# swusjask/kzg-snark

Hardware: AMD Instinct MI355X
Metric: KZG G1 commits/sec (INTT 2^20 + commit 2^20, BLS12-381) (higher is better)
Workload: dtype integer: 13x30-bit limbs in u32 (381-bit Fp), 9x29-bit limbs (255-bit Fr), 64-bit multiply-add; 1 GPU; degree-2^20 INTT + KZG commit, bls12_381, 2^20-point SRS, uniform Fr scalars, batch of 4 polynomials per GPU per step; log_n=20, curve=bls12_381, batch=4, window_bits=20

## Files before the change

### kzg_snark_amd/csrc/api.hip

```cpp
#include "internal.h"
#include "g1_words.h"
#include "msm.h"
#include "../../include/kzg_mi355x.h"
#include <cstdio>
#include <cstring>
#include <new>

struct kzg_ctx {
  kzg::Ctx c;
};
struct kzg_srs {
  kzg::Srs* s;
};
struct kzg_domain_table {
  kzg::DomainTable* t;
};

namespace kzg {
int device_any_nonzero(Ctx* c, const uint32_t* d_words, size_t from, size_t to, bool* out);
}

namespace kzg {

int set_err(Ctx* c, int code, const char* what, hipError_t e) {
  if (c) {
    c->err = what ? what : "";
    if (e != hipSuccess) {
      c->err += ": ";
      c->err += hipGetErrorString(e);
    }
  }
  return code;
}

ProfScope::ProfScope(Ctx* ctx, const char* name, hipStream_t stream) : c(ctx) {
  if (!c->prof_on) return;
  st = stream ? stream : c->stream;
  for (auto& sp : c->prof)
    if (sp.name == name) { span = &sp; break; }
  if (!span) {
    c->prof.reserve(64);
    c->prof.push_back(ProfSpan{name, {}, 0, 0});
    span = &c->prof.back();
  }
  if (hipEventCreate(&e0) != hipSuccess || hipEventCreate(&e1) != hipSuccess) { span = nullptr; return; }
  hipEventRecord(e0, st);
}
ProfScope::~ProfScope() {
  if (!span) return;
  hipEventRecord(e1, st);
  span->pending.emplace_back(e0, e1);
}

int ensure_buf(Ctx* c, DevBuf& b, size_t bytes) {
  if (b.cap >= bytes) return KZG_OK;
  if (b.p) {
    KZG_HIP(c, hipStreamSynchronize(c->stream));
    KZG_HIP(c, hipFree(b.p));
    b.p = nullptr;
    b.cap = 0;
  }
  hipError_t e = hipMalloc(&b.p, bytes);
  if (e != hipSuccess) {
    b.p = nullptr;
    return set_err(c, KZG_ERR_ALLOC, "hipMalloc", e);
  }
  b.cap = bytes;
  return KZG_OK;
}

}

namespace kzg {
template <class C>
static int g1_sum_t(const uint64_t* xy, const uint8_t* inf, size_t n, uint64_t* out_xy, uint8_t* out_inf) {
  using F = typename C::Fp;
  const uint32_t* w = reinterpret_cast<const uint32_t*>(xy);
  XYZZ<C> acc = Ec<C>::infinity();
  for (size_t i = 0; i < n; ++i) {
    if (inf && inf[i]) continue;
    Fe<F> x, y;
    if (!import_affine<C>(w + i * 2 * F::NW, w + i * 2 * F::NW + F::NW, x, y)) return KZG_ERR_ARG;
    acc = Ec<C>::madd(acc, x, y);
  }
  *out_inf = affine_to_words<C>(Ec<C>::to_affine(acc), reinterpret_cast<uint32_t*>(out_xy));
  return KZG_OK;
}
}

using namespace kzg;

#define KZG_ENTER(bad)                           \
  if (!ctx || (bad)) return KZG_ERR_ARG;         \
  Ctx* c = &ctx->c;                              \
  KZG_HIP(c, hipSetDevice(c->device))

static int adopt_srs(int rc, Srs* s, kzg_srs** out) {
  if (rc == KZG_OK) *out = new kzg_srs{s};
  return rc;
}

static int stage_host(Ctx* c, const void* src, size_t bytes, void** d) {
  int rc = ensure_buf(c, c->io, bytes ? bytes : 32);
  if (rc) return rc;
  if (bytes) KZG_HIP(c, hipMemcpyAsync(c->io.p, src, bytes, hipMemcpyHostToDevice, c->stream));
  *d = c->io.p;
  return KZG_OK;
}

extern "C" {

int kzg_g1_sum(int curve_id, const uint64_t* xy, const uint8_t* inf, size_t n, uint64_t* out_xy, uint8_t* out_inf) {
  if ((n && !xy) || !out_xy || !out_inf) return KZG_ERR_ARG;
  if (curve_id == KZG_CURVE_BN254) return g1_sum_t<Bn254>(xy, inf, n, out_xy, out_inf);
  if (curve_id == KZG_CURVE_BLS12_381) return g1_sum_t<Bls12_381>(xy, inf, n, out_xy, out_inf);
  return KZG_ERR_ARG;
}

int kzg_abi_version(void) { return 1; }

int kzg_fp_limbs(int curve_id) {
  if (curve_id == KZG_CURVE_BN254) return 4;
  if (curve_id == KZG_CURVE_BLS12_381) return 6;
  return 0;
}

int kzg_ctx_create(int curve_id, int device_id, kzg_ctx** out) {
  if (!out) return KZG_ERR_ARG;
  *out = nullptr;
  if (curve_id != KZG_CURVE_BN254 && curve_id != KZG_CURVE_BLS12_381) return KZG_ERR_ARG;
  int ndev = 0;
  if (hipGetDeviceCount(&ndev) != hipSuccess || ndev <= 0 || device_id < 0 || device_id >= ndev)
    return KZG_ERR_NODEV;
  if (hipSetDevice(device_id) != hipSuccess) return KZG_ERR_NODEV;
  kzg_ctx* h = new (std::nothrow) kzg_ctx();
  if (!h) return KZG_ERR_ALLOC;
  h->c.curve = curve_id;
  h->c.device = device_id;
  if (hipStreamCreateWithFlags(&h->c.stream, hipStreamNonBlocking) != hipSuccess) {
    delete h;
    return KZG_ERR_HIP;
  }
  h->c.own_stream = true;
  *out = h;
  return KZG_OK;
}

void kzg_ctx_destroy(kzg_ctx* ctx) {
  if (!ctx) return;
  Ctx* c = &ctx->c;
  hipSetDevice(c->device);
  hipDeviceSynchronize();
  ntt_free_domains(c);
  msm_free_work(c);
  for (DevBuf* b : {&c->ntt_scratch, &c->io, &c->scan_tmp, &c->lagr_tmp, &c->dom_tmp, &c->ver_tmp, &c->rec_tmp,
                    &c->vpt_tmp, &c->pair_tmp, &c->gmul_tmp,
                    &c->poly_tmp[0], &c->poly_tmp[1], &c->poly_tmp[2], &c->poly_tmp[3]})
    hipFree(b->p);
  hipFree(c->clk_probe);
  if (c->eval_lens_pin) hipHostFree(c->eval_lens_pin);
  if (c->eval_lens_ev) hipEventDestroy(c->eval_lens_ev);
  for (auto s : c->aux_streams) hipStreamDestroy(s);
  for (auto e : c->aux_events) hipEventDestroy(e);
  if (c->own_stream && c->stream) hipStreamDestroy(c->stream);
  delete ctx;
}

const char* kzg_last_error(const kzg_ctx* ctx) { return ctx ? ctx->c.err.c_str() : "null context"; }

int kzg_ctx_set_stream(kzg_ctx* ctx, void* hip_stream) {
  KZG_ENTER(false);
  if (hip_stream) {
    const uintptr_t hv = reinterpret_cast<uintptr_t>(hip_stream);
    const bool alias = hip_stream == static_cast<void*>(hipStreamLegacy) || hip_stream == static_cast<void*>(hipStreamPerThread);
    if (!alias && (hv < 65536 || (hv & 7)))
      return set_err(c, KZG_ERR_ARG, "kzg_ctx_set_stream: not a stream handle (small integer or misaligned value)");
    if (c->own_stream && c->stream) {
      KZG_HIP(c, hipStreamSynchronize(c->stream));
      KZG_HIP(c, hipStreamDestroy(c->stream));
    }
    c->stream = hip_stream == static_cast<void*>(hipStreamLegacy) ? nullptr : static_cast<hipStream_t>(hip_stream);
    c->own_stream = false;
  } else if (!c->own_stream) {
    KZG_HIP(c, hipStreamCreateWithFlags(&c->stream, hipStreamNonBlocking));
    c->own_stream = true;
  }
  return KZG_OK;
}

int kzg_ctx_set_tuning(kzg_ctx* ctx, const char* key, int64_t value) {
  if (!ctx || !key) return KZG_ERR_ARG;
  Ctx* c = &ctx->c;
  const std::string k(key);
  if (k == "ntt_tile_log") {
    if (value != 0 && (value < 8 || value > 12)) return set_err(c, KZG_ERR_ARG, "ntt_tile_log: 0 or 8..12");
    c->tune_ntt_tile_log = (int)value;
  } else if (k == "open_tile_threads") {
    if (value != 0 && value != 128 && value != 256) return set_err(c, KZG_ERR_ARG, "open_tile_threads: 0, 128 or 256");
    c->tune_open_tb = (int)value;
  } else if (k == "open_direct_tiles") {
    if (value < 0 || value > (1 << 20)) return set_err(c, KZG_ERR_ARG, "open_direct_tiles: 0 .. 2^20");
    c->tune_open_direct_max = (int)value;
  } else if (k == "open_domain_chunk") {
    if (value < 0 || value > 1024) return set_err(c, KZG_ERR_ARG, "open_domain_chunk: 0 .. 1024");
    c->tune_open_domain_chunk = (int)value;
  } else if (k == "open_cosets_chunk") {
    if (value < 0 || value > 1024) return set_err(c, KZG_ERR_ARG, "open_cosets_chunk: 0 .. 1024");
    c->tune_open_cosets_chunk = (int)value;
  } else if (k == "open_cosets_group") {
    if (value < 0 || value > 5) return set_err(c, KZG_ERR_ARG, "open_cosets_group: 0 .. 5");
    c->tune_open_cosets_group = (int)value;
  } else if (k == "recover_chunk") {
    if (value < 0 || value > 1024) return set_err(c, KZG_ERR_ARG, "recover_chunk: 0 .. 1024");
    c->tune_recover_chunk = (int)value;
  } else if (k == "eval_batch_chunk") {
    if (value < 0 || value > 65535) return set_err(c, KZG_ERR_ARG, "eval_batch_chunk: 0 .. 65535");
    c->tune_eval_batch_chunk = (int)value;
  } else {
    return set_err(c, KZG_ERR_ARG, "kzg_ctx_set_tuning: unknown key");
  }
  return KZG_OK;
}

int kzg_ctx_synchronize(kzg_ctx* ctx) {
  if (!ctx) return KZG_ERR_ARG;
  Ctx* c = &ctx->c;
  KZG_HIP(c, hipStreamSynchronize(c->stream));
  return KZG_OK;
}

int kzg_ntt_device(kzg_ctx* ctx, void* d_data, uint32_t log_n, const uint64_t w[4], int inverse,
                   uint32_t batch) {
  KZG_ENTER(!d_data || !w);
  return ntt_run_device(c, static_cast<uint32_t*>(d_data), log_n, reinterpret_cast<const uint32_t*>(w),
                        inverse ? 1 : 0, batch);
}

int kzg_ntt_columns_device(kzg_ctx* ctx, void* d_data, uint32_t log_n, const uint64_t w[4], int inverse,
                           uint64_t n_cols, uint64_t col_base) {
  KZG_ENTER(!d_data || !w);
  return ntt_partial_device(c, static_cast<uint32_t*>(d_data), log_n, reinterpret_cast<const uint32_t*>(w),
                            inverse ? 1 : 0, 0, n_cols, col_base);
}

int kzg_ntt_rows_device(kzg_ctx* ctx, void* d_data, uint32_t log_n, const uint64_t w[4], int inverse,
                        uint64_t n_rows) {
  KZG_ENTER(!d_data || !w);
  return ntt_partial_device(c, static_cast<uint32_t*>(d_data), log_n, reinterpret_cast<const uint32_t*>(w),
                            inverse ? 1 : 0, 1, n_rows, 0);
}

int kzg_ntt_rows_twist_device(kzg_ctx* ctx, void* d_data, uint32_t log_n, const uint64_t w[4], int inverse,
                              uint64_t n_rows, uint64_t row_base) {
  KZG_ENTER(!d_data || !w);
  return ntt_partial_device(c, static_cast<uint32_t*>(d_data), log_n, reinterpret_cast<const uint32_t*>(w),
                            inverse ? 1 : 0, 2, n_rows, row_base);
}

int kzg_ntt_columns_plain_device(kzg_ctx* ctx, void* d_data, uint32_t log_n, const uint64_t w[4], int inverse,
                                 uint64_t n_cols) {
  KZG_ENTER(!d_data || !w);
  return ntt_partial_device(c, static_cast<uint32_t*>(d_data), log_n, reinterpret_cast<const uint32_t*>(w),
                            inverse ? 1 : 0, 3, n_cols, 0);
}

int kzg_ntt_rows_exchange_device(kzg_ctx* ctx, const void* d_src, void* d_dst, uint32_t log_n, const uint64_t w[4],
                                 int inverse, uint64_t n_rows, uint32_t world, int blocked_out) {
  KZG_ENTER(!d_src || !d_dst || !w);
  return ntt_rows_exchange_device(c, static_cast<const uint32_t*>(d_src), static_cast<uint32_t*>(d_dst), log_n,
                                  reinterpret_cast<const uint32_t*>(w), inverse ? 1 : 0, n_rows, world, blocked_out);
}

int kzg_ntt(kzg_ctx* ctx, uint64_t* data, uint32_t log_n, const uint64_t w[4], int inverse) {
  KZG_ENTER(!data || !w);
  if (log_n > 24) return set_err(c, KZG_ERR_ARG, "kzg_ntt: log_n > 24 not supported");
  const size_t bytes = (size_t)32 << log_n;
  void* d = nullptr;
  int rc = stage_host(c, data, bytes, &d);
  if (rc) return rc;
  rc = ntt_run_device(c, static_cast<uint32_t*>(d), log_n, reinterpret_cast<const uint32_t*>(w), inverse ? 1 : 0, 1);
  if (rc) return rc;
  KZG_HIP(c, hipMemcpyAsync(data, d, bytes, hipMemcpyDeviceToHost, c->stream));
  KZG_HIP(c, hipStreamSynchronize(c->stream));
  return KZG_OK;
}

int kzg_fft_ff_any_device(kzg_ctx* ctx, void* d_data, size_t n, const uint64_t w[4], int inverse) {
  KZG_ENTER(!d_data || !w);
  if (n && !(n & (n - 1))) {
    uint32_t log_n = 0;
    while ((1ull << log_n) < n) ++log_n;
    return ntt_run_device(c, static_cast<uint32_t*>(d_data), log_n, reinterpret_cast<const uint32_t*>(w),
                          inverse ? 1 : 0, 1);
  }
  return fft_ragged_device(c, static_cast<uint32_t*>(d_data), n, reinterpret_cast<const uint32_t*>(w), inverse ? 1 : 0);
}

int kzg_fft_ff_any(kzg_ctx* ctx, uint64_t* data, size_t n, const uint64_t w[4], int inverse) {
  KZG_ENTER(!data || !w);
  if (n == 0 || n > ((size_t)1 << 24)) return set_err(c, KZG_ERR_ARG, "kzg_fft_ff_any: length must be in [1, 2^24]");
  const size_t bytes = n * 32;
  void* d = nullptr;
  int rc = stage_host(c, data, bytes, &d);
  if (rc) return rc;
  rc = kzg_fft_ff_any_device(ctx, d, n, w, inverse);
  if (rc) return rc;
  KZG_HIP(c, hipMemcpyAsync(data, d, bytes, hipMemcpyDeviceToHost, c->stream));
  KZG_HIP(c, hipStreamSynchronize(c->stream));
  return KZG_OK;
}

int kzg_srs_load_g1(kzg_ctx* ctx, const uint64_t* xy, const uint8_t* inf, size_t n, kzg_srs** out) {
  KZG_ENTER(!xy || !out);
  *out = nullptr;
  Srs* s = nullptr;
  const int rc = srs_load(c, xy, inf, n, &s);
  return adopt_srs(rc, s, out);
}

int kzg_srs_generate_range(kzg_ctx* ctx, const uint64_t tau[4], size_t start, size_t n, kzg_srs** out) {
  KZG_ENTER(!tau || !out);
  *out = nullptr;
  Srs* s = nullptr;
  const int rc = srs_generate(c, tau, start, n, &s);
  return adopt_srs(rc, s, out);
}

int kzg_srs_generate_strided(kzg_ctx* ctx, const uint64_t tau[4], size_t start, size_t n, size_t run_len,
                             size_t inner_stride, size_t outer_stride, kzg_srs** out) {
  KZG_ENTER(!tau || !out || run_len == 0);
  *out = nullptr;
  Srs* s = nullptr;
  const int rc = srs_generate(c, tau, start, n, &s, run_len, inner_stride, outer_stride);
  return adopt_srs(rc, s, out);
}

int kzg_srs_generate(kzg_ctx* ctx, const uint64_t tau[4], size_t n, kzg_srs** out) {
  return kzg_srs_generate_range(ctx, tau, 0, n, out);
}

int kzg_srs_export(kzg_ctx* ctx, const kzg_srs* srs, size_t start, size_t count, uint64_t* xy, uint8_t* inf) {
  KZG_ENTER(!srs || !xy || !inf);
  return srs_export(c, srs->s, start, count, xy, inf);
}

int kzg_srs_load_g1_compressed(kzg_ctx* ctx, const uint8_t* bytes, size_t n, int check_subgroup, kzg_srs** out) {
  KZG_ENTER(!bytes || !out);
  *out = nullptr;
  Srs* s = nullptr;
  const int rc = srs_load_g1_compressed(c, bytes, n, check_subgroup, &s);
  return adopt_srs(rc, s, out);
}

int kzg_srs_export_compressed(kzg_ctx* ctx, const kzg_srs* srs, size_t start, size_t count, uint8_t* out_bytes) {
  KZG_ENTER(!srs || (count && !out_bytes));
  if (srs->s->curve != c->curve) return set_err(c, KZG_ERR_ARG, "SRS belongs to another curve");
  return srs_export_compressed(c, srs->s, start, count, out_bytes);
}

int kzg_g1_compress(kzg_ctx* ctx, const uint64_t* xy, const uint8_t* inf, size_t n, uint8_t* out_bytes) {
  KZG_ENTER(n && (!xy || !out_bytes));
  return g1_compress(c, xy, inf, n, out_bytes);
}

int kzg_g1_decompress(kzg_ctx* ctx, const uint8_t* bytes, size_t n, int check_subgroup, uint64_t* out_xy,
                      uint8_t* out_inf, uint8_t* out_status) {
  KZG_ENTER(n && (!bytes || !out_xy || !out_inf || !out_status));
  return g1_decompress(c, bytes, n, check_subgroup, out_xy, out_inf, out_status);
}

int kzg_g1_decompress_device(kzg_ctx* ctx, const void* d_bytes, size_t n, int check_subgroup, void* d_xy, void* d_inf,
                             void* d_status) {
  KZG_ENTER(n && (!d_bytes || !d_xy || !d_inf || !d_status));
  return g1_decompress_device(c, d_bytes, n, check_subgroup, d_xy, d_inf, d_status);
}

int kzg_g1_check_subgroup(kzg_ctx* ctx, const uint64_t* xy, const uint8_t* inf, size_t n, uint8_t* out_status) {
  KZG_ENTER(n && (!xy || !out_status));
  return g1_check_subgroup(c, xy, inf, n, out_status);
}

int kzg_g2_compress(kzg_ctx* ctx, const uint64_t* xy, const uint8_t* inf, size_t n, uint8_t* out_bytes) {
  KZG_ENTER(n && (!xy || !out_bytes));
  return g2_compress(c, xy, inf, n, out_bytes);
}

int kzg_g2_decompress(kzg_ctx* ctx, const uint8_t* bytes, size_t n, int check_subgroup, uint64_t* out_xy,
                      uint8_t* out_inf, uint8_t* out_status) {
  KZG_ENTER(n && (!bytes || !out_xy || !out_inf || !out_status));
  return g2_decompress(c, bytes, n, check_subgroup, out_xy, out_inf, out_status);
}

int kzg_g2_decompress_device(kzg_ctx* ctx, const void* d_bytes, size_t n, int check_subgroup, void* d_xy, void* d_inf,
                             void* d_status) {
  KZG_ENTER(n && (!d_bytes || !d_xy || !d_inf || !d_status));
  return g2_decompress_device(c, d_bytes, n, check_subgroup, d_xy, d_inf, d_status);
}

int kzg_g2_check_subgroup(kzg_ctx* ctx, const uint64_t* xy, const uint8_t* inf, size_t n, uint8_t* out_status) {
  KZG_ENTER(n && (!xy || !out_status));
  return g2_check_subgroup(c, xy, inf, n, out_status);
}

int kzg_g1_mul_each(kzg_ctx* ctx, const uint64_t* xy, const uint8_t* inf, size_t n, const uint64_t* scalars,
                    uint64_t* out_xy, uint8_t* out_inf) {
  KZG_ENTER(n && (!xy || !scalars || !out_xy || !out_inf));
  return g1_mul_each(c, xy, inf, n, reinterpret_cast<const uint32_t*>(scalars), nullptr, nullptr, out_xy, out_inf);
}

int kzg_g1_mul_each_device(kzg_ctx* ctx, const void* d_xy, const void* d_inf, size_t n, const void* d_scalars,
                           void* d_out_xy, void* d_out_inf) {
  KZG_ENTER(n && (!d_xy || !d_scalars || !d_out_xy || !d_out_inf));
  return g1_mul_each_device(c, d_xy, d_inf, n, d_scalars, d_out_xy, d_out_inf);
}

int kzg_g1_mul_powers(kzg_ctx* ctx, const uint64_t* xy, const uint8_t* inf, size_t n, const uint64_t s[4],
                      const uint64_t c0[4], uint64_t* out_xy, uint8_t* out_inf) {
  KZG_ENTER(!s || !c0 || (n && (!xy || !out_xy || !out_inf)));
  return g1_mul_each(c, xy, inf, n, nullptr, reinterpret_cast<const uint32_t*>(s), reinterpret_cast<const uint32_t*>(c0),
                     out_xy, out_inf);
}

int kzg_srs_mul_powers(kzg_ctx* ctx, const kzg_srs* srs, const uint64_t s[4], const uint64_t c0[4], kzg_srs** out) {
  KZG_ENTER(!srs || !s || !c0 || !out);
  *out = nullptr;
  if (srs->s->curve != c->curve) return set_err(c, KZG_ERR_ARG, "SRS belongs to another curve");
  Srs* key = nullptr;
  const int rc = srs_mul_powers(c, srs->s, reinterpret_cast<const uint32_t*>(s), reinterpret_cast<const uint32_t*>(c0), &key);
  return adopt_srs(rc, key, out);
}

int kzg_g2_mul_each(kzg_ctx* ctx, const uint64_t* xy, const uint8_t* inf, size_t n, const uint64_t* scalars,
                    uint64_t* out_xy, uint8_t* out_inf) {
  KZG_ENTER(n && (!xy || !scalars || !out_xy || !out_inf));
  return g2_mul_each(c, xy, inf, n, reinterpret_cast<const uint32_t*>(scalars), nullptr, nullptr, out_xy, out_inf);
}

int kzg_g2_mul_powers(kzg_ctx* ctx, const uint64_t* xy, const uint8_t* inf, size_t n, const uint64_t s[4],
                      const uint64_t c0[4], uint64_t* out_xy, uint8_t* out_inf) {
  KZG_ENTER(!s || !c0 || (n && (!xy || !out_xy || !out_inf)));
  return g2_mul_each(c, xy, inf, n, nullptr, reinterpret_cast<const uint32_t*>(s), reinterpret_cast<const uint32_t*>(c0),
                     out_xy, out_inf);
}

int kzg_g2_lincomb(kzg_ctx* ctx, const uint64_t* xy, const uint8_t* inf, size_t n, const uint64_t* scalars,
                   uint64_t* out_xy, uint8_t* out_inf) {
  KZG_ENTER(!out_xy || !out_inf || (n && (!xy || !scalars)));
  return g2_lincomb(c, xy, inf, n, reinterpret_cast<const uint32_t*>(scalars), nullptr, nullptr, out_xy, out_inf);
}

int kzg_g2_lincomb_powers(kzg_ctx* ctx, const uint64_t* xy, const uint8_t* inf, size_t n, const uint64_t s[4],
                          const uint64_t c0[4], uint64_t* out_xy, uint8_t* out_inf) {
  KZG_ENTER(!s || !c0 || !out_xy || !out_inf || (n && !xy));
  return g2_lincomb(c, xy, inf, n, nullptr, reinterpret_cast<const uint32_t*>(s), reinterpret_cast<const uint32_t*>(c0),
                    out_xy, out_inf);
}

int kzg_pairing_check(kzg_ctx* ctx, const uint64_t* g1_xy, const uint8_t* g1_inf, const uint64_t* g2_xy,
                      const uint8_t* g2_inf, size_t m, size_t k, uint8_t* out_status) {
  KZG_ENTER(m && (!g1_xy || !g2_xy || !out_status));
  return pairing_product(c, g1_xy, g1_inf, g2_xy, g2_inf, m, k, nullptr, out_status);
}

int kzg_pairing_product(kzg_ctx* ctx, const uint64_t* g1_xy, const uint8_t* g1_inf, const uint64_t* g2_xy,
                        const uint8_t* g2_inf, size_t m, size_t k, uint64_t* out_gt, uint8_t* out_status) {
  KZG_ENTER(m && (!g1_xy || !g2_xy || !out_gt || !out_status));
  return pairing_product(c, g1_xy, g1_inf, g2_xy, g2_inf, m, k, out_gt, out_status);
}

int kzg_pairing_gt_multiple(int curve) { return pairing_gt_multiple(curve); }

int kzg_blob_to_fr(kzg_ctx* ctx, uint32_t log_n, const uint8_t* blobs, size_t b, int bit_reversed, uint64_t* out_vals,
                   uint8_t* out_status) {
  KZG_ENTER(b && (!blobs || !out_vals || !out_status));
  return blob_to_fr(c, log_n, blobs, b, bit_reversed, out_vals, out_status);
}

int kzg_blob_to_fr_device(kzg_ctx* ctx, uint32_t log_n, const void* d_blobs, size_t b, int bit_reversed, void* d_vals,
                          void* d_status) {
  KZG_ENTER(b && (!d_blobs || !d_vals || !d_status));
  return blob_to_fr_device(c, log_n, d_blobs, b, bit_reversed, d_vals, d_status);
}

int kzg_fr_to_blob(kzg_ctx* ctx, uint32_t log_n, const uint64_t* vals, size_t b, int bit_reversed, uint8_t* out_bytes,
                   uint8_t* out_status) {
  KZG_ENTER(b && (!vals || !out_bytes || !out_status));
  return fr_to_blob(c, log_n, vals, b, bit_reversed, out_bytes, out_status);
}

int kzg_fr_to_blob_device(kzg_ctx* ctx, uint32_t log_n, const void* d_vals, size_t b, int bit_reversed, void* d_bytes,
                          void* d_status) {
  KZG_ENTER(b && (!d_vals || !d_bytes || !d_status));
  return fr_to_blob_device(c, log_n, d_vals, b, bit_reversed, d_bytes, d_status);
}

int kzg_blob_challenges(kzg_ctx* ctx, uint32_t log_n, const uint8_t* blobs, const uint8_t* commitments, size_t b,
                        uint64_t* out_z) {
  KZG_ENTER(b && (!blobs || !commitments || !out_z));
  return blob_challenges(c, log_n, blobs, commitments, b, out_z);
}

int kzg_blob_challenges_device(kzg_ctx* ctx, uint32_t log_n, const void* d_blobs, const void* d_commitments, size_t b,
                               void* d_z) {
  KZG_ENTER(b && (!d_blobs || !d_commitments || !d_z));
  return blob_challenges_device(c, log_n, d_blobs, d_commitments, b, d_z);
}

size_t kzg_srs_size(const kzg_srs* srs) { return srs ? srs->s->n : 0; }

void kzg_srs_free(kzg_srs* srs) {
  if (!srs) return;
  srs_free(srs->s);
  delete srs;
}

int kzg_commit_device(kzg_ctx* ctx, const kzg_srs* srs, const void* d_scalars, const size_t* lens, size_t n_polys,
                      size_t stride, uint64_t* out_xy, uint8_t* out_inf) {
  KZG_ENTER(!srs || !lens || !out_xy || !out_inf || (n_polys && !d_scalars));
  return commit_device(c, srs->s, static_cast<const uint32_t*>(d_scalars), lens, n_polys, stride, out_xy, out_inf);
}

int kzg_commit_device_async(kzg_ctx* ctx, const kzg_srs* srs, const void* d_scalars, const size_t* lens,
                            size_t n_polys, size_t stride, uint64_t* out_xy, uint8_t* out_inf) {
  KZG_ENTER(!srs || !lens || !out_xy || !out_inf || (n_polys && !d_scalars));
  return commit_device(c, srs->s, static_cast<const uint32_t*>(d_scalars), lens, n_polys, stride, out_xy, out_inf,
                       false);
}

int kzg_commit_flush(kzg_ctx* ctx) {
  KZG_ENTER(false);
  return commit_flush(c);
}

int kzg_commit(kzg_ctx* ctx, const kzg_srs* srs, const uint64_t* scalars, const size_t* lens, size_t n_polys,
               size_t stride, uint64_t* out_xy, uint8_t* out_inf) {
  KZG_ENTER(!srs || !lens || !out_xy || !out_inf || (n_polys && stride && !scalars));
  const size_t bytes = n_polys * stride * 32;
  int rc = ensure_buf(c, c->io, bytes ? bytes : 32);
  if (rc) return rc;
  const size_t fpw = (c->curve == 0 ? Bn254::Fp::NW : Bls12_381::Fp::NW) / 2;
  auto* io = static_cast<uint32_t*>(c->io.p);
  for (size_t p = 0; p < n_polys; ++p) {
    if (lens[p] > srs->s->n) return set_err(c, KZG_ERR_DEGREE, "polynomial longer than the commitment key");
    if (lens[p] > stride) return set_err(c, KZG_ERR_ARG, "kzg_commit: lens[p] > stride");
  }
  for (size_t p = 0; p < n_polys && rc == KZG_OK; ++p) {
    if (lens[p])
      rc = KZG_HIP_RC(c, hipMemcpyAsync(io + p * stride * 8, scalars + p * stride * 4, lens[p] * 32,
                                        hipMemcpyHostToDevice, c->stream));
    if (rc == KZG_OK)
      rc = commit_device(c, srs->s, io + p * stride * 8, lens + p, 1, stride, out_xy + p * 2 * fpw, out_inf + p, false);
  }
  const int rc2 = commit_flush(c);
  return rc ? rc : rc2;
}

int kzg_open_device(kzg_ctx* ctx, const kzg_srs* srs, const void* d_polys, const size_t* lens, size_t k,
                    size_t stride, const uint64_t z[4], const uint64_t xi[4], uint64_t* out_xy, uint8_t* out_inf,
                    uint64_t* eval_out) {
  KZG_ENTER(!srs || !z || !xi || !out_xy || !out_inf || (k && (!lens || !d_polys)));
  uint32_t* d_quot = nullptr;
  size_t qlen = 0;
  uint64_t ev[4];
  int rc = open_quotient_device(c, static_cast<const uint32_t*>(d_polys), lens, k, stride,
                                reinterpret_cast<const uint32_t*>(z), reinterpret_cast<const uint32_t*>(xi), &d_quot,
                                &qlen, ev);
  if (rc) return rc;
  if (eval_out) memcpy(eval_out, ev, 32);
  const size_t srs_n = srs->s->n;
  if (qlen > srs_n) {
    bool nz = false;
    rc = device_any_nonzero(c, d_quot, srs_n, qlen, &nz);
    if (rc) return rc;
    if (nz) return set_err(c, KZG_ERR_DEGREE, "witness polynomial longer than the commitment key");
    qlen = srs_n;
  }
  return commit_device(c, srs->s, d_quot, &qlen, 1, qlen ? qlen : 1, out_xy, out_inf);
}

int kzg_open_device_async(kzg_ctx* ctx, const kzg_srs* srs, const void* d_polys, const size_t* lens, size_t k,
                          size_t stride, const uint64_t z[4], const uint64_t xi[4], uint64_t* out_xy, uint8_t* out_inf,
                          uint64_t* eval_out) {
  KZG_ENTER(!srs || !z || !xi || !out_xy || !out_inf || !eval_out || (k && (!lens || !d_polys)));
  uint32_t* d_quot = nullptr;
  size_t qlen = 0;
  int rc = open_quotient_device(c, static_cast<const uint32_t*>(d_polys), lens, k, stride,
                                reinterpret_cast<const uint32_t*>(z), reinterpret_cast<const uint32_t*>(xi), &d_quot,
                                &qlen, eval_out, false);
  if (rc) return rc;
  if (!d_quot) {
    memset(out_xy, 0, (size_t)kzg_fp_limbs(c->curve) * 16);
    *out_inf = 1;
    memset(eval_out, 0, 32);
    return KZG_OK;
  }
  const size_t srs_n = srs->s->n;
  if (qlen > srs_n) {
    bool nz = false;
    rc = device_any_nonzero(c, d_quot, srs_n, qlen, &nz);
    if (rc) return rc;
    if (nz) return set_err(c, KZG_ERR_DEGREE, "witness polynomial longer than the commitment key");
    qlen = srs_n;
  }
  return commit_device(c, srs->s, d_quot, &qlen, 1, qlen ? qlen : 1, out_xy, out_inf, false, d_quot - 8,
                       eval_out);
}

int kzg_open(kzg_ctx* ctx, const kzg_srs* srs, const uint64_t* polys, const size_t* lens, size_t k, size_t stride,
             const uint64_t z[4], const uint64_t xi[4], uint64_t* out_xy, uint8_t* out_inf, uint64_t* eval_out) {
  KZG_ENTER(!srs || !z || !xi || !out_xy || !out_inf || (k && (!lens || !polys)));
  void* d = nullptr;
  if (int rc = stage_host(c, polys, k * stride * 32, &d)) return rc;
  return kzg_open_device(ctx, srs, d, lens, k, stride, z, xi, out_xy, out_inf, eval_out);
}

int kzg_open_points_device(kzg_ctx* ctx, const kzg_srs* srs, const void* d_polys, const size_t* lens, size_t k,
                           size_t stride, const uint64_t* points, size_t t, const uint64_t* weights, void* d_quot,
                           uint64_t* out_xy, uint8_t* out_inf) {
  KZG_ENTER(!srs || !out_xy || !out_inf || (k && (!lens || !d_polys)) || (t && !points) || (k && t && !weights));
  uint32_t* d_q = nullptr;
  size_t qlen = 0;
  int rc = open_points_quotient_device(c, static_cast<const uint32_t*>(d_polys), lens, k, stride,
                                       reinterpret_cast<const uint32_t*>(points), t,
                                       reinterpret_cast<const uint32_t*>(weights), &d_q, &qlen);
  if (rc) return rc;
  if (!d_q) {
    memset(out_xy, 0, (size_t)kzg_fp_limbs(c->curve) * 16);
    *out_inf = 1;
    return KZG_OK;
  }
  if (d_quot) KZG_HIP(c, hipMemcpyAsync(d_quot, d_q, qlen * 32, hipMemcpyDeviceToDevice, c->stream));
  const size_t srs_n = srs->s->n;
  if (qlen > srs_n) {
    bool nz = false;
    rc = device_any_nonzero(c, d_q, srs_n, qlen, &nz);
    if (rc) return rc;
    if (nz) return set_err(c, KZG_ERR_DEGREE, "witness polynomial longer than the commitment key");
    qlen = srs_n;
  }
  return commit_device(c, srs->s, d_q, &qlen, 1, qlen ? qlen : 1, out_xy, out_inf);
}

int kzg_open_points(kzg_ctx* ctx, const kzg_srs* srs, const uint64_t* polys, const size_t* lens, size_t k,
                    size_t stride, const uint64_t* points, size_t t, const uint64_t* weights, void* d_quot,
                    uint64_t* out_xy, uint8_t* out_inf) {
  KZG_ENTER(!srs || !out_xy || !out_inf || (k && (!lens || !polys)));
  void* d = nullptr;
  if (int rc = stage_host(c, polys, k * stride * 32, &d)) return rc;
  return kzg_open_points_device(ctx, srs, d, lens, k, stride, points, t, weights, d_quot, out_xy, out_inf);
}

int kzg_open_shard_begin(kzg_ctx* ctx, const void* d_polys, const size_t* lens, size_t k, size_t stride,
                         const uint64_t z[4], const uint64_t xi[4], uint64_t* chunk_eval_out) {
  KZG_ENTER(!z || !xi || !chunk_eval_out || (k && (!lens || !d_polys)));
  return open_shard_begin_device(c, static_cast<const uint32_t*>(d_polys), lens, k, stride,
                                 reinterpret_cast<const uint32_t*>(z), reinterpret_cast<const uint32_t*>(xi),
                                 chunk_eval_out);
}

int kzg_open_shard_finish(kzg_ctx* ctx, const kzg_srs* srs, const uint64_t z[4], const uint64_t carry[4],
                          int first_rank, uint64_t* out_xy, uint8_t* out_inf, uint64_t* eval_out) {
  KZG_ENTER(!srs || !z || !carry || !out_xy || !out_inf);
  uint32_t* d_vec = nullptr;
  size_t len = 0;
  uint64_t ev[4];
  int rc = open_shard_finish_device(c, reinterpret_cast<const uint32_t*>(z), reinterpret_cast<const uint32_t*>(carry),
                                    first_rank, &d_vec, &len, ev);
  if (rc) return rc;
  if (eval_out) memcpy(eval_out, ev, 32);
  if (len > srs->s->n) return set_err(c, KZG_ERR_DEGREE, "quotient slice longer than the key shard");
  return commit_device(c, srs->s, d_vec, &len, 1, len ? len : 1, out_xy, out_inf);
}

int kzg_srs_generate_lagrange(kzg_ctx* ctx, const uint64_t tau[4], uint32_t log_n, const uint64_t w[4],
                              kzg_srs** out) {
  KZG_ENTER(!tau || !w || !out);
  *out = nullptr;
  Srs* s = nullptr;
  const int rc = srs_generate_lagrange(c, reinterpret_cast<const uint32_t*>(tau), log_n, reinterpret_cast<const uint32_t*>(w),
                                 &s);
  return adopt_srs(rc, s, out);
}

int kzg_srs_lagrange(kzg_ctx* ctx, const kzg_srs* monomial, uint32_t log_n, const uint64_t w[4], kzg_srs** out) {
  KZG_ENTER(!monomial || !w || !out);
  *out = nullptr;
  Srs* s = nullptr;
  const int rc = srs_lagrange(c, monomial->s, log_n, reinterpret_cast<const uint32_t*>(w), &s);
  return adopt_srs(rc, s, out);
}

int kzg_open_evals_device(kzg_ctx* ctx, const kzg_srs* srs, const void* d_vals, const size_t* lens, size_t k,
                          size_t stride, const uint64_t z[4], const uint64_t xi[4], uint64_t* out_xy, uint8_t* out_inf,
                          uint64_t* eval_out) {
  KZG_ENTER(!srs || !z || !xi || !out_xy || !out_inf || (k && (!lens || !d_vals)));
  return open_evals_device(c, srs->s, static_cast<const uint32_t*>(d_vals), lens, k, stride,
                           reinterpret_cast<const uint32_t*>(z), reinterpret_cast<const uint32_t*>(xi), out_xy, out_inf,
                           eval_out, true);
}

int kzg_open_evals_device_async(kzg_ctx* ctx, const kzg_srs* srs, const void* d_vals, const size_t* lens, size_t k,
                                size_t stride, const uint64_t z[4], const uint64_t xi[4], uint64_t* out_xy,
                                uint8_t* out_inf, uint64_t* eval_out) {
  KZG_ENTER(!srs || !z || !xi || !out_xy || !out_inf || !eval_out || (k && (!lens || !d_vals)));
  return open_evals_device(c, srs->s, static_cast<const uint32_t*>(d_vals), lens, k, stride,
                           reinterpret_cast<const uint32_t*>(z), reinterpret_cast<const uint32_t*>(xi), out_xy, out_inf,
                           eval_out, false);
}

int kzg_open_evals(kzg_ctx* ctx, const kzg_srs* srs, const uint64_t* vals, const size_t* lens, size_t k, size_t stride,
                   const uint64_t z[4], const uint64_t xi[4], uint64_t* out_xy, uint8_t* out_inf, uint64_t* eval_out) {
  KZG_ENTER(!srs || !z || !xi || !out_xy || !out_inf || (k && (!lens || !vals)));
  void* d = nullptr;
  if (int rc = stage_host(c, vals, k * stride * 32, &d)) return rc;
  return kzg_open_evals_device(ctx, srs, d, lens, k, stride, z, xi, out_xy, out_inf, eval_out);
}

int kzg_domain_table_create(kzg_ctx* ctx, const kzg_srs* monomial, uint32_t log_n, kzg_domain_table** out) {
  KZG_ENTER(!monomial || !out);
  *out = nullptr;
  DomainTable* t = nullptr;
  int rc = domain_table_create(c, monomial->s, log_n, &t);
  if (rc) return rc;
  *out = new kzg_domain_table{t};
  return KZG_OK;
}

size_t kzg_domain_table_size(const kzg_domain_table* t) { return t ? domain_table_size(t->t) : 0; }

void kzg_domain_table_free(kzg_domain_table* t) {
  if (!t) return;
  domain_table_free(t->t);
  delete t;
}

int kzg_open_domain_device(kzg_ctx* ctx, const kzg_domain_table* t, const void* d_polys, const size_t* lens, size_t b,
                           size_t stride, const uint64_t w[4], uint64_t* out_xy, uint8_t* out_inf,
                           uint64_t* eval_out) {
  KZG_ENTER(!t || !w || (b && (!lens || !d_polys || !out_xy || !out_inf)));
  return open_domain(c, t->t, static_cast<const uint32_t*>(d_polys), false, lens, b, stride,
                     reinterpret_cast<const uint32_t*>(w), out_xy, out_inf, eval_out);
}

int kzg_open_domain(kzg_ctx* ctx, const kzg_domain_table* t, const uint64_t* polys, const size_t* lens, size_t b,
                    size_t stride, const uint64_t w[4], uint64_t* out_xy, uint8_t* out_inf, uint64_t* eval_out) {
  KZG_ENTER(!t || !w || (b && (!lens || !polys || !out_xy || !out_inf)));
  return open_domain(c, t->t, reinterpret_cast<const uint32_t*>(polys), true, lens, b, stride,
                     reinterpret_cast<const uint32_t*>(w), out_xy, out_inf, eval_out);
}

int kzg_coset_table_create(kzg_ctx* ctx, const kzg_srs* monomial, uint32_t log_n, uint32_t log_l,
                           kzg_domain_table** out) {
  KZG_ENTER(!monomial || !out);
  *out = nullptr;
  DomainTable* t = nullptr;
  int rc = coset_table_create(c, monomial->s, log_n, log_l, &t);
  if (rc) return rc;
  *out = new kzg_domain_table{t};
  return KZG_OK;
}

int kzg_open_cosets_device(kzg_ctx* ctx, const kzg_domain_table* t, const void* d_polys, const size_t* lens, size_t b,
                           size_t stride, uint32_t log_N, const uint64_t w[4], uint64_t* out_xy, uint8_t* out_inf,
                           uint64_t* eval_out) {
  KZG_ENTER(!t || !w || (b && (!lens || !d_polys || !out_xy || !out_inf)));
  return open_cosets(c, t->t, static_cast<const uint32_t*>(d_polys), false, lens, b, stride, log_N,
                     reinterpret_cast<const uint32_t*>(w), out_xy, out_inf, eval_out);
}

int kzg_open_cosets(kzg_ctx* ctx, const kzg_domain_table* t, const uint64_t* polys, const size_t* lens, size_t b,
                    size_t stride, uint32_t log_N, const uint64_t w[4], uint64_t* out_xy, uint8_t* out_inf,
                    uint64_t* eval_out) {
  KZG_ENTER(!t || !w || (b && (!lens || !polys || !out_xy || !out_inf)));
  return open_cosets(c, t->t, reinterpret_cast<const uint32_t*>(polys), true, lens, b, stride, log_N,
                     reinterpret_cast<const uint32_t*>(w), out_xy, out_inf, eval_out);
}

int kzg_open_coset_device(kzg_ctx* ctx, const kzg_srs* srs, const void* d_polys, const size_t* lens, size_t k,
                          size_t stride, uint32_t log_l, const uint64_t h[4], const uint64_t zeta[4],
                          const uint64_t xi[4], uint64_t* out_xy, uint8_t* out_inf, uint64_t* eval_out) {
  KZG_ENTER(!srs || !h || !zeta || !xi || !out_xy || !out_inf || (k && (!lens || !d_polys)));
  if (srs->s->curve != c->curve) return set_err(c, KZG_ERR_ARG, "SRS belongs to another curve");
  if (srs->s->basis != SRS_MONOMIAL) return set_err(c, KZG_ERR_ARG, "kzg_open_coset: the key must be monomial");
  uint32_t* d_quot = nullptr;
  size_t qlen = 0;
  int rc = open_coset_quotient_device(c, static_cast<const uint32_t*>(d_polys), lens, k, stride, log_l,
                                      reinterpret_cast<const uint32_t*>(h), reinterpret_cast<const uint32_t*>(zeta),
                                      reinterpret_cast<const uint32_t*>(xi), srs->s->n, &d_quot, &qlen, eval_out);
  if (rc) return rc;
  return commit_device(c, srs->s, d_quot, &qlen, 1, qlen ? qlen : 1, out_xy, out_inf);
}

int kzg_open_coset(kzg_ctx* ctx, const kzg_srs* srs, const uint64_t* polys, const size_t* lens, size_t k,
                   size_t stride, uint32_t log_l, const uint64_t h[4], const uint64_t zeta[4], const uint64_t xi[4],
                   uint64_t* out_xy, uint8_t* out_inf, uint64_t* eval_out) {
  KZG_ENTER(!srs || !h || !zeta || !xi || !out_xy || !out_inf || (k && (!lens || !polys)));
  if (srs->s->curve != c->curve) return set_err(c, KZG_ERR_ARG, "SRS belongs to another curve");
  if (srs->s->basis != SRS_MONOMIAL) return set_err(c, KZG_ERR_ARG, "kzg_open_coset: the key must be monomial");
  int rc = open_coset_check(c, lens, k, stride, log_l, reinterpret_cast<const uint32_t*>(h),
                            reinterpret_cast<const uint32_t*>(zeta), srs->s->n);
  if (rc) return rc;
  void* d = nullptr;
  if ((rc = stage_host(c, polys, k * stride * 32, &d))) return rc;
  return kzg_open_coset_device(ctx, srs, d, lens, k, stride, log_l, h, zeta, xi, out_xy, out_inf, eval_out);
}

int kzg_verify_cosets(kzg_ctx* ctx, const kzg_srs* monomial, uint32_t log_N, uint32_t log_l, const uint64_t w[4],
                      const uint64_t* comm_xy, const uint8_t* comm_inf, size_t n_comm, const uint32_t* comm_idx,
                      const uint32_t* coset_idx, const uint64_t* values, const uint64_t* proof_xy,
                      const uint8_t* proof_inf, size_t K, const uint64_t rho[4], uint64_t* out_xy, uint8_t* out_inf) {
  KZG_ENTER(!monomial || !w || !rho || !out_xy || !out_inf || !comm_xy || (K && (!comm_idx || !coset_idx ||
            !values || !proof_xy)));
  return verify_cosets(c, monomial->s, log_N, log_l, reinterpret_cast<const uint32_t*>(w), comm_xy, comm_inf, n_comm,
                       comm_idx, coset_idx, values, proof_xy, proof_inf, K, reinterpret_cast<const uint32_t*>(rho),
                       out_xy, out_inf);
}

int kzg_verify_cosets_bytes(kzg_ctx* ctx, const kzg_srs* monomial, uint32_t log_N, uint32_t log_l, const uint64_t w[4],
                            const uint64_t* comm_xy, const uint8_t* comm_inf, size_t n_comm, const uint32_t* comm_idx,
                            const uint32_t* coset_idx, const uint8_t* cells, int bit_reversed, const uint64_t* proof_xy,
                            const uint8_t* proof_inf, size_t K, const uint64_t rho[4], uint64_t* out_xy,
                            uint8_t* out_inf, uint8_t* out_status) {
  KZG_ENTER(!monomial || !w || !rho || !out_xy || !out_inf || !out_status || !comm_xy || (K && (!comm_idx ||
            !coset_idx || !cells || !proof_xy)));
  return verify_cosets_bytes(c, monomial->s, log_N, log_l, reinterpret_cast<const uint32_t*>(w), comm_xy, comm_inf,
                             n_comm, comm_idx, coset_idx, cells, bit_reversed, proof_xy, proof_inf, K,
                             reinterpret_cast<const uint32_t*>(rho), out_xy, out_inf, out_status);
}

int kzg_verify_points(kzg_ctx* ctx, const uint64_t* comm_xy, const uint8_t* comm_inf, size_t n_comm,
                      const uint32_t* comm_idx, const uint64_t* z, const uint64_t* y, const uint64_t* proof_xy,
                      const uint8_t* proof_inf, size_t K, const uint64_t rho[4], uint64_t* out_xy, uint8_t* out_inf) {
  KZG_ENTER(!rho || !out_xy || !out_inf || !comm_xy || (K && (!comm_idx || !z || !y || !proof_xy)));
  return verify_points(c, comm_xy, comm_inf, n_comm, comm_idx, z, y, proof_xy, proof_inf, K,
                       reinterpret_cast<const uint32_t*>(rho), out_xy, out_inf);
}

int kzg_recover_cosets(kzg_ctx* ctx, uint32_t log_n, uint32_t log_N, uint32_t log_l, const uint64_t w[4],
                       const uint32_t* coset_idx, size_t K, const uint64_t* values, size_t b, uint64_t* out_coeffs,
                       uint8_t* out_consistent) {
  KZG_ENTER(!w || !coset_idx || !values || !out_coeffs || !out_consistent);
  return recover_cosets(c, log_n, log_N, log_l, reinterpret_cast<const uint32_t*>(w), coset_idx, K,
                        reinterpret_cast<const uint32_t*>(values), true, b,
                        reinterpret_cast<uint32_t*>(out_coeffs), out_consistent);
}

int kzg_recover_cosets_device(kzg_ctx* ctx, uint32_t log_n, uint32_t log_N, uint32_t log_l, const uint64_t w[4],
                              const uint32_t* coset_idx, size_t K, const void* d_values, size_t b, void* d_coeffs,
                              uint8_t* out_consistent) {
  KZG_ENTER(!w || !coset_idx || !d_values || !d_coeffs || !out_consistent);
  return recover_cosets(c, log_n, log_N, log_l, reinterpret_cast<const uint32_t*>(w), coset_idx, K,
                        static_cast<const uint32_t*>(d_values), false, b,
                        static_cast<uint32_t*>(d_coeffs), out_consistent);
}

int kzg_fr_vec_op(kzg_ctx* ctx, int op, size_t n, const void* d_a, const void* d_b, void* d_out) {
  KZG_ENTER(false);
  if (op < 0 || op > 2 || (n && (!d_a || !d_b || !d_out))) return KZG_ERR_ARG;
  return fr_vec_binary(c, op, n, static_cast<const uint32_t*>(d_a), static_cast<const uint32_t*>(d_b),
                       static_cast<uint32_t*>(d_out));
}

int kzg_fr_vec_lincomb(kzg_ctx* ctx, size_t n, size_t k, const void* const* d_ptrs, const size_t* lens,
                       const uint64_t* scalars, void* d_out) {
  KZG_ENTER(false);
  if (k && (!d_ptrs || !lens || !scalars)) return KZG_ERR_ARG;
  if (n && !d_out) return KZG_ERR_ARG;
  return fr_vec_lincomb(c, n, k, reinterpret_cast<const uint32_t* const*>(d_ptrs), lens,
                        reinterpret_cast<const uint32_t*>(scalars), static_cast<uint32_t*>(d_out));
}

int kzg_fr_vec_mul_powers(kzg_ctx* ctx, size_t n, const void* d_a, const uint64_t s[4], const uint64_t c0[4],
                          void* d_out) {
  KZG_ENTER(false);
  if (!s || !c0 || (n && (!d_a || !d_out))) return KZG_ERR_ARG;
  return fr_vec_mul_powers(c, n, static_cast<const uint32_t*>(d_a), reinterpret_cast<const uint32_t*>(s),
                           reinterpret_cast<const uint32_t*>(c0), static_cast<uint32_t*>(d_out));
}

int kzg_fr_vec_inverse(kzg_ctx* ctx, size_t n, const void* d_a, void* d_out) {
  KZG_ENTER(false);
  if (n && (!d_a || !d_out)) return KZG_ERR_ARG;
  return fr_vec_inverse(c, n, static_cast<const uint32_t*>(d_a), static_cast<uint32_t*>(d_out));
}

int kzg_fr_vec_prefix_product(kzg_ctx* ctx, size_t n, const void* d_a, void* d_out) {
  KZG_ENTER(false);
  if (n && (!d_a || !d_out)) return KZG_ERR_ARG;
  return fr_vec_prefix_product(c, n, static_cast<const uint32_t*>(d_a), static_cast<uint32_t*>(d_out));
}

int kzg_fr_poly_eval(kzg_ctx* ctx, size_t n, const void* d_a, const uint64_t z[4], uint64_t out[4]) {
  KZG_ENTER(false);
  if (!z || !out || (n && !d_a)) return KZG_ERR_ARG;
  return fr_poly_eval(c, n, static_cast<const uint32_t*>(d_a), reinterpret_cast<const uint32_t*>(z), out);
}

int kzg_fr_poly_eval_batch(kzg_ctx* ctx, const void* d_polys, const size_t* lens, size_t k, size_t stride,
                           const uint64_t* points, size_t t, uint64_t* out) {
  KZG_ENTER(false);
  if (k && t && (!d_polys || !lens || !points || !out)) return KZG_ERR_ARG;
  return fr_poly_eval_batch(c, static_cast<const uint32_t*>(d_polys), lens, k, stride,
                            reinterpret_cast<const uint32_t*>(points), t, out);
}

int kzg_fr_eval_lagrange(kzg_ctx* ctx, uint32_t log_n, const uint64_t w[4], size_t len, const void* d_vals,
                         const uint64_t z[4], uint64_t out[4]) {
  KZG_ENTER(false);
  if (!w || !z || !out || (len && !d_vals)) return KZG_ERR_ARG;
  return fr_eval_lagrange(c, log_n, reinterpret_cast<const uint32_t*>(w), len, static_cast<const uint32_t*>(d_vals),
                          reinterpret_cast<const uint32_t*>(z), out);
}

int kzg_fr_eval_lagrange_batch_device(kzg_ctx* ctx, uint32_t log_n, const uint64_t w[4], const void* d_vals,
                                      const size_t* lens, size_t b, size_t stride, const void* d_z, void* d_out) {
  KZG_ENTER(false);
  if (!w || (b && (!d_vals || !lens || !d_z || !d_out))) return KZG_ERR_ARG;
  return fr_eval_lagrange_batch(c, log_n, reinterpret_cast<const uint32_t*>(w), static_cast<const uint32_t*>(d_vals),
                                lens, b, stride, static_cast<const uint32_t*>(d_z), static_cast<uint32_t*>(d_out));
}

int kzg_fr_eval_lagrange_batch(kzg_ctx* ctx, uint32_t log_n, const uint64_t w[4], const uint64_t* vals,
                               const size_t* lens, size_t b, size_t stride, const uint64_t* z, uint64_t* out) {
  KZG_ENTER(false);
  if (!w || (b && (!vals || !lens || !z || !out))) return KZG_ERR_ARG;
  if (b == 0) return KZG_OK;
  if (stride == 0 || b > ((size_t)1 << 40) / stride) return set_err(c, KZG_ERR_ARG, "kzg_fr_eval_lagrange_batch: b * stride too large");
  const size_t vb = b * stride * 32, zb = b * 32;
  int rc = ensure_buf(c, c->io, vb + 2 * zb);
  if (rc) return rc;
  char* d = static_cast<char*>(c->io.p);
  KZG_HIP(c, hipMemcpyAsync(d, vals, vb, hipMemcpyHostToDevice, c->stream));
  KZG_HIP(c, hipMemcpyAsync(d + vb, z, zb, hipMemcpyHostToDevice, c->stream));
  rc = kzg_fr_eval_lagrange_batch_device(ctx, log_n, w, d, lens, b, stride, d + vb, d + vb + zb);
  if (rc) return rc;
  KZG_HIP(c, hipMemcpyAsync(out, d + vb + zb, zb, hipMemcpyDeviceToHost, c->stream));
  KZG_HIP(c, hipStreamSynchronize(c->stream));
  return KZG_OK;
}

int kzg_prof_enable(kzg_ctx* ctx, int on) {
  if (!ctx) return KZG_ERR_ARG;
  Ctx* c = &ctx->c;
  if (on && !c->clk_probe) {
    KZG_HIP(c, hipMalloc(reinterpret_cast<void**>(&c->clk_probe), CLK_WORDS * 8));
    KZG_HIP(c, hipMemset(c->clk_probe, 0, CLK_WORDS * 8));
  }
  c->prof_on = on != 0;
  return KZG_OK;
}

int kzg_prof_reset(kzg_ctx* ctx) {
  if (!ctx) return KZG_ERR_ARG;
  Ctx* c = &ctx->c;
  KZG_HIP(c, hipDeviceSynchronize());
  for (auto& sp : c->prof) {
    for (auto& pr : sp.pending) { hipEventDestroy(pr.first); hipEventDestroy(pr.second); }
    sp.pending.clear();
    sp.total_ms = 0;
    sp.count = 0;
  }
  if (c->clk_probe) KZG_HIP(c, hipMemset(c->clk_probe, 0, CLK_WORDS * 8));
  return KZG_OK;
}

int kzg_prof_read(kzg_ctx* ctx, const char* name, double* total_ms, uint64_t* count) {
  if (!ctx || !name || !total_ms || !count) return KZG_ERR_ARG;
  Ctx* c = &ctx->c;
  KZG_HIP(c, hipDeviceSynchronize());
  *total_ms = 0;
  *count = 0;
  const bool acc_clk = std::string(name) == "msm_accumulate_shader_mhz", ntt_clk = std::string(name) == "ntt_pass_shader_mhz";
  if (std::string(name) == "verify_device_bytes") {
    *total_ms = (double)c->ver_last_bytes;
    *count = c->ver_last_bytes ? 1 : 0;
    return KZG_OK;
  }
  if (std::string(name) == "verify_points_device_bytes") {
    *total_ms = (double)c->vpt_last_bytes;
    *count = c->vpt_last_bytes ? 1 : 0;
    return KZG_OK;
  }
  if (std::string(name) == "recover_leaf") {
    *total_ms = (double)recover_leaf_width();
    *count = 1;
    return KZG_OK;
  }
  if (std::string(name) == "ntt_tile_log") {
    *total_ms = (double)c->last_ntt_tile_log;
    *count = c->last_ntt_tile_log ? 1 : 0;
    return KZG_OK;
  }
  const bool acc_tail = std::string(name) == "msm_accumulate_tail_us", acc_spread = std::string(name) == "msm_accumulate_exit_spread_us";
  if (acc_tail || acc_spread) {
    unsigned long long t[CLK_WORDS] = {0};
    if (c->clk_probe) KZG_HIP(c, hipMemcpy(t, c->clk_probe, sizeof(t), hipMemcpyDeviceToHost));
    const unsigned long long waves = t[CLK_ACC_WAVES], launches = t[CLK_ACC_LAUNCHES];
    if (launches && waves) {
      const unsigned long long ticks = acc_tail ? (waves * t[CLK_ACC_EXIT_LAST] - t[CLK_ACC_EXIT_SUM]) / waves
                                                : t[CLK_ACC_EXIT_LAST] - t[CLK_ACC_EXIT_FIRST];
      *total_ms = (double)ticks / 100.0 / (double)launches;
      *count = launches;
    }
    return KZG_OK;
  }
  if (acc_clk || ntt_clk) {
    unsigned long long t[4] = {0, 0, 0, 0};
    if (c->clk_probe) KZG_HIP(c, hipMemcpy(t, c->clk_probe, 32, hipMemcpyDeviceToHost));
    const unsigned long long* q = t + (ntt_clk ? 2 : 0);
    if (q[1]) { *total_ms = 100.0 * (double)q[0] / (double)q[1]; *count = 1; }
    return KZG_OK;
  }
  for (auto& sp : c->prof) {
    if (sp.name != name) continue;
    for (auto& pr : sp.pending) {
      float ms = 0;
      if (hipEventElapsedTime(&ms, pr.first, pr.second) == hipSuccess) { sp.total_ms += ms; sp.count += 1; }
      hipEventDestroy(pr.first);
      hipEventDestroy(pr.second);
    }
    sp.pending.clear();
    *total_ms = sp.total_ms;
    *count = sp.count;
    return KZG_OK;
  }
  return KZG_OK;
}

}
```

### kzg_snark_amd/csrc/internal.h

```cpp
#pragma once
#include <hip/hip_runtime.h>
#include <stdint.h>
#include <stddef.h>
#include <string>
#include <vector>
#include "field.h"
#include "devmem.h"

namespace kzg {

constexpr int KZG_OK = 0;
constexpr int KZG_ERR_ARG = -1;
constexpr int KZG_ERR_HIP = -2;
constexpr int KZG_ERR_NODEV = -3;
constexpr int KZG_ERR_DEGREE = -4;
constexpr int KZG_ERR_ALLOC = -5;

struct NttDomain {
  uint32_t log_n = 0;
  int inverse = 0;
  uint32_t w[8] = {0};
  uint32_t kmax = 0;
  uint32_t h = 0;
  uint32_t* d_stage = nullptr;
  uint32_t* d_twA = nullptr;
  uint32_t* d_twB = nullptr;
  uint32_t* d_scale = nullptr;
  uint32_t* d_twist = nullptr;
  uint64_t last_use = 0;
};

struct ProfSpan {
  std::string name;
  std::vector<std::pair<hipEvent_t, hipEvent_t>> pending;
  double total_ms = 0;
  uint64_t count = 0;
};

enum : int {
  CLK_ACC_LAUNCHES = 4,
  CLK_ACC_EXIT_SUM = 5,
  CLK_ACC_EXIT_FIRST = 6,
  CLK_ACC_EXIT_LAST = 7,
  CLK_ACC_WAVES = 8,
  CLK_WORDS = 16
};

struct TileShape {
  size_t n = 0;
  uint32_t tb = 0, ntiles = 0, nsuper = 0;
  uint32_t *G = nullptr, *H = nullptr, *A = nullptr, *zinv = nullptr, *W = nullptr;
  uint32_t z[9] = {0}, z_inv[9] = {0};
};
struct OpenSlice {
  enum State { NEVER, HELD, LOST } state = NEVER;
  uint32_t z_words[8] = {0};
  TileShape shape;
};

struct Ctx {
  int curve = 0;
  int device = 0;
  hipStream_t stream = nullptr;
  bool own_stream = false;
  std::string err;
  std::vector<NttDomain> domains;
  uint64_t tick = 0;
  uint32_t ntt_lds_attr_set = 0;
  DevBuf ntt_scratch;
  DevBuf io;
  DevBuf poly_tmp[4];
  DevBuf scan_tmp;
  DevBuf lagr_tmp;
  DevBuf dom_tmp;
  DevBuf ver_tmp;
  DevBuf rec_tmp;
  DevBuf vpt_tmp;
  DevBuf pair_tmp;
  DevBuf gmul_tmp;
  size_t ver_last_bytes = 0;
  size_t vpt_last_bytes = 0;
  uint32_t ver_lds_attr_set = 0;
  uint32_t* eval_lens_pin = nullptr;
  size_t eval_lens_cap = 0;
  hipEvent_t eval_lens_ev = nullptr;
  OpenSlice open_slice;
  int tune_ntt_tile_log = 0;
  int tune_open_tb = 0;
  int tune_open_direct_max = 0;
  int tune_open_domain_chunk = 0;
  int tune_open_cosets_chunk = 0;
  int tune_open_cosets_group = 0;
  int tune_recover_chunk = 0;
  int tune_eval_batch_chunk = 0;
  int last_ntt_tile_log = 0;
  void* msm_work = nullptr;
  bool prof_on = false;
  std::vector<ProfSpan> prof;
  unsigned long long* clk_probe = nullptr;
  std::vector<hipStream_t> aux_streams;
  std::vector<hipEvent_t> aux_events;
};

int set_err(Ctx* c, int code, const char* what, hipError_t e = hipSuccess);
struct ProfScope {
  Ctx* c;
  ProfSpan* span = nullptr;
  hipEvent_t e0 = nullptr, e1 = nullptr;
  hipStream_t st = nullptr;
  ProfScope(Ctx* ctx, const char* name, hipStream_t stream = nullptr);
  ~ProfScope();
};

#define KZG_HIP(c, call)                                         \
  do {                                                           \
    hipError_t e__ = (call);                                     \
    if (e__ != hipSuccess) return set_err((c), KZG_ERR_HIP, #call, e__); \
  } while (0)
#define KZG_HIP_RC(c, call) hip_rc((c), (call), #call)
inline int hip_rc(Ctx* c, hipError_t e, const char* what) { return e == hipSuccess ? KZG_OK : set_err(c, KZG_ERR_HIP, what, e); }

#define KZG_BY_CURVE(c, fn, ...) ((c)->curve == 0 ? fn<Bn254>(__VA_ARGS__) : fn<Bls12_381>(__VA_ARGS__))
#define KZG_BY_FR(c, fn, ...) ((c)->curve == 0 ? fn<BnFr>(__VA_ARGS__) : fn<BlsFr>(__VA_ARGS__))

bool msm_accumulate_in_flight(Ctx* c);

int ntt_run_device(Ctx* c, uint32_t* d_data, uint32_t log_n, const uint32_t* w_words, int inverse,
                   uint32_t batch);
int ntt_partial_device(Ctx* c, uint32_t* d_data, uint32_t log_n, const uint32_t* w_words, int inverse, int rows_pass,
                       uint64_t count, uint64_t col_base);
int ntt_rows_exchange_device(Ctx* c, const uint32_t* d_src, uint32_t* d_dst, uint32_t log_n, const uint32_t* w_words,
                             int inverse, uint64_t n_rows, uint32_t world, int blocked_out);
int fft_ragged_device(Ctx* c, uint32_t* d_data, uint64_t n, const uint32_t* w_words, int inverse);
void ntt_free_domains(Ctx* c);

int fr_vec_binary(Ctx* c, int op, size_t n, const uint32_t* a, const uint32_t* b, uint32_t* out);
int fr_vec_lincomb(Ctx* c, size_t n, size_t k, const uint32_t* const* ptrs, const size_t* lens, const uint32_t* scalars,
                   uint32_t* out);
int fr_vec_mul_powers(Ctx* c, size_t n, const uint32_t* a, const uint32_t* s, const uint32_t* cc, uint32_t* out);
int fr_vec_inverse(Ctx* c, size_t n, const uint32_t* a, uint32_t* out);
int fr_vec_prefix_product(Ctx* c, size_t n, const uint32_t* a, uint32_t* out);
int fr_poly_eval(Ctx* c, size_t n, const uint32_t* a, const uint32_t* z, uint64_t* out);
int fr_poly_eval_batch(Ctx* c, const uint32_t* d_polys, const size_t* lens, size_t k, size_t stride,
                       const uint32_t* points, size_t t, uint64_t* out);

struct FrArg;
__attribute__((visibility("hidden")))
int fr_pow_table(Ctx* c, const FrArg& base, uint32_t* d_tab);

}
```

### kzg_snark_amd/csrc/msm.hip

```cpp
#include <cstring>
#include <cstdlib>
#include <string.h>
#include <algorithm>
#include <vector>
#include <type_traits>
#include <utility>
#include "internal.h"
#include "ec.h"
#include "msm.h"
#include "msm_prep.h"
#include "srs_rec.h"
#include "g1_words.h"

namespace kzg {

namespace {

template <int WB>
struct Win {
  static constexpr int BITS = WB;
  static constexpr int NWIN = (256 + WB - 1) / WB;
  static constexpr uint32_t NB = 1u << (WB - 1);
  static constexpr uint32_t SEG = WB >= 20 ? 64 : 32;
  static constexpr uint32_t FIN = WB >= 20 ? 2 : 8;
  static constexpr int LO = WB / 2;
  static constexpr int HI = WB - 1 - LO;
  static constexpr int NPART = HI + LO + 1;
};
constexpr int MAX_NPART = 24;

template <class C>
__device__ __forceinline__ XYZZ<C> load_xyzz(const uint32_t* base, size_t idx) {
  constexpr int N = C::Fp::N;
  static_assert((4 * N) % 4 == 0, "XYZZ must be a whole number of quads");
  const uint4* p = reinterpret_cast<const uint4*>(base + idx * 4 * N);
  uint32_t w[4 * N];
#pragma unroll
  for (int q = 0; q < N; ++q) {
    const uint4 v = p[q];
    w[4 * q] = v.x; w[4 * q + 1] = v.y; w[4 * q + 2] = v.z; w[4 * q + 3] = v.w;
  }
  XYZZ<C> r;
#pragma unroll
  for (int j = 0; j < N; ++j) { r.x.l[j] = w[j]; r.y.l[j] = w[N + j]; r.zz.l[j] = w[2 * N + j]; r.zzz.l[j] = w[3 * N + j]; }
  return r;
}
template <class C>
__device__ __forceinline__ void store_xyzz(uint32_t* base, size_t idx, const XYZZ<C>& v) {
  constexpr int N = C::Fp::N;
  uint32_t w[4 * N];
#pragma unroll
  for (int j = 0; j < N; ++j) { w[j] = v.x.l[j]; w[N + j] = v.y.l[j]; w[2 * N + j] = v.zz.l[j]; w[3 * N + j] = v.zzz.l[j]; }
  uint4* p = reinterpret_cast<uint4*>(base + idx * 4 * N);
#pragma unroll
  for (int q = 0; q < N; ++q) p[q] = make_uint4(w[4 * q], w[4 * q + 1], w[4 * q + 2], w[4 * q + 3]);
}
template <class C>
__device__ __forceinline__ XYZZ<C> shfl_xor_xyzz(const XYZZ<C>& v, int mask) {
  constexpr int N = C::Fp::N;
  XYZZ<C> r;
#pragma unroll
  for (int j = 0; j < N; ++j) {
    r.x.l[j] = __shfl_xor(v.x.l[j], mask);
    r.y.l[j] = __shfl_xor(v.y.l[j], mask);
    r.zz.l[j] = __shfl_xor(v.zz.l[j], mask);
    r.zzz.l[j] = __shfl_xor(v.zzz.l[j], mask);
  }
  return r;
}


template <class C, bool RANGE>
__global__ __launch_bounds__(256) void g1_import_kernel(const uint32_t* xy, const uint8_t* inf, uint32_t* recs, size_t n,
                                                        uint32_t* bad) {
  using F = typename C::Fp;
  const size_t i = (size_t)blockIdx.x * blockDim.x + threadIdx.x;
  if (i >= n) return;
  Affine<C> a = affine_from_words<C>(nullptr, true);
  a.inf = inf && inf[i];
  if (!a.inf) {
    uint32_t w[2 * F::NW];
#pragma unroll
    for (int k = 0; k < 2 * F::NW; ++k) w[k] = xy[i * 2 * F::NW + k];
    bool ok;
    if constexpr (RANGE) {
      ok = import_affine<C>(w, w + F::NW, a.x, a.y);
    } else {
      a = affine_from_words<C>(w, false);
      ok = Ec<C>::on_curve(a.x, a.y);
    }
    if (!ok) atomicAdd(bad, 1u);
  }
  store_rec<C>(recs, i, a.x, a.y, a.inf);
}

template <class C>
__global__ __launch_bounds__(128) void srs_window_kernel(const uint32_t* src, uint32_t* dst, size_t n, int win_bits) {
  using F = typename C::Fp;
  using Fd = Field<F>;
  const size_t i = (size_t)blockIdx.x * blockDim.x + threadIdx.x;
  if (i >= n) return;
  Fe<F> x, y;
  load_rec<C>(src, i, x, y);
  const bool is_inf = src[i * Rec<C>::WORDS + Rec<C>::FLAG] & 1u;
  XYZZ<C> p = is_inf ? Ec<C>::infinity() : Ec<C>::dbl_affine(x, y);
  for (int d = 1; d < win_bits; ++d) p = Ec<C>::dbl(p);
  const Affine<C> a = Ec<C>::to_affine(p);
  store_rec<C>(dst, i, Fd::reduce(a.x), Fd::reduce(a.y), a.inf);
}

template <class C>
__global__ void srs_export_kernel(const uint32_t* recs, size_t start, size_t count, uint32_t* xy, uint8_t* inf) {
  using F = typename C::Fp;
  const size_t i = (size_t)blockIdx.x * blockDim.x + threadIdx.x;
  if (i >= count) return;
  Affine<C> a;
  load_rec<C>(recs, start + i, a.x, a.y);
  a.inf = recs[(start + i) * Rec<C>::WORDS + Rec<C>::FLAG] & 1u;
  uint32_t w[2 * F::NW];
  inf[i] = affine_to_words<C>(a, w) ? 1 : 0;
#pragma unroll
  for (int k = 0; k < 2 * F::NW; ++k) xy[i * 2 * F::NW + k] = w[k];
}

template <class C>
__global__ __launch_bounds__(256) void gen_table_kernel(const uint32_t* g_rec, uint32_t* tab) {
  using F = typename C::Fp;
  using Fd = Field<F>;
  const uint32_t j = blockIdx.x;
  const uint32_t d = threadIdx.x + 1;
  if (d > 255) return;
  Fe<F> gx, gy;
  load_rec<C>(g_rec, 0, gx, gy);
  XYZZ<C> base;
  base.x = gx; base.y = gy; base.zz = Fd::one(); base.zzz = Fd::one();
  for (uint32_t q = 0; q < 8 * j; ++q) base = Ec<C>::dbl(base);
  XYZZ<C> acc = Ec<C>::infinity();
  for (int bit = 7; bit >= 0; --bit) {
    acc = Ec<C>::dbl(acc);
    if ((d >> bit) & 1u) acc = Ec<C>::add(acc, base);
  }
  const Affine<C> a = Ec<C>::to_affine(acc);
  store_rec<C>(tab, (size_t)j * 255 + (d - 1), Fd::reduce(a.x), Fd::reduce(a.y), a.inf);
}

template <class C>
__global__ __launch_bounds__(128) void srs_generate_kernel(const uint32_t* tab, const uint32_t* tau_mont,
                                                           uint32_t* recs, size_t start, size_t n, size_t run_len,
                                                           size_t inner_stride, size_t outer_stride,
                                                           const uint32_t* scalars) {
  using F = typename C::Fp;
  using Fr = typename C::Fr;
  using Fd = Field<F>;
  using Frd = Field<Fr>;
  const size_t i = (size_t)blockIdx.x * blockDim.x + threadIdx.x;
  if (i >= n) return;
  uint32_t s[Fr::NW];
  if (scalars) {
#pragma unroll
    for (int j = 0; j < Fr::NW; ++j) s[j] = scalars[i * Fr::NW + j];
  } else {
    Fe<Fr> b, acc = Frd::one();
#pragma unroll
    for (int j = 0; j < Fr::N; ++j) b.l[j] = tau_mont[j];
    for (size_t bits = start + (i / run_len) * outer_stride + (i % run_len) * inner_stride; bits; bits >>= 1) {
      if (bits & 1u) acc = Frd::mul(acc, b);
      b = Frd::mul(b, b);
    }
    Frd::to_words(Frd::from_mont(acc), s);
  }
  XYZZ<C> p = Ec<C>::infinity();
  for (int j = 0; j < 32; ++j) {
    const uint32_t d = (s[j >> 2] >> (8 * (j & 3))) & 0xffu;
    if (d) {
      Fe<F> x, y;
      load_rec<C>(tab, (size_t)j * 255 + (d - 1), x, y);
      p = Ec<C>::madd(p, x, y);
    }
  }
  const Affine<C> a = Ec<C>::to_affine(p);
  store_rec<C>(recs, i, Fd::reduce(a.x), Fd::reduce(a.y), a.inf);
}


template <class C>
struct RecStage {
  static constexpr int N = C::Fp::N;
  static constexpr int Q = (2 * N + 1 + 3) / 4;
  static constexpr int WAVE_WORDS = Q * 64 * 4;
  static_assert(4 * Q <= Rec<C>::WORDS && (Rec<C>::WORDS % 4) == 0, "records are whole 16-byte quads");

  static __device__ __forceinline__ void issue(const uint32_t* recs, uint32_t idx, uint32_t* stage) {
    const uint32_t* src = recs + (size_t)idx * Rec<C>::WORDS;
    issue_quads(src, stage, std::make_integer_sequence<int, Q>());
  }
  template <int... Qs>
  static __device__ __forceinline__ void issue_quads(const uint32_t* src, uint32_t* stage,
                                                     std::integer_sequence<int, Qs...>) {
    (__builtin_amdgcn_global_load_lds(src, (__attribute__((address_space(3))) uint32_t*)(stage + Qs * (256 - 4)), 16,
                                      16 * Qs, 0),
     ...);
  }
  static __device__ __forceinline__ uint32_t read(const uint32_t* stage, uint32_t lane, Fe<typename C::Fp>& x,
                                                  Fe<typename C::Fp>& y) {
    uint32_t w[4 * Q];
#pragma unroll
    for (int q = 0; q < Q; ++q) {
      const uint4 t = *reinterpret_cast<const uint4*>(stage + q * 256 + lane * 4);
      w[4 * q] = t.x; w[4 * q + 1] = t.y; w[4 * q + 2] = t.z; w[4 * q + 3] = t.w;
    }
#pragma unroll
    for (int j = 0; j < N; ++j) { x.l[j] = w[j]; y.l[j] = w[N + j]; }
    return w[Rec<C>::FLAG];
  }
};

template <class C, int WB>
__global__ __launch_bounds__(128, 3) void msm_accumulate_kernel(const uint32_t* recs, const uint32_t* vals,
                                                             const uint32_t* bstart, const uint32_t* order,
                                                             const uint32_t* slice_off, uint32_t* partials,
                                                             uint32_t* buckets, uint32_t* chunk_counter,
                                                             const uint32_t* chunk_rank, unsigned long long* clk) {
  using F = typename C::Fp;
  using Fd = Field<F>;
  using St = RecStage<C>;
  constexpr uint32_t NB = Win<WB>::NB;
  __shared__ __attribute__((aligned(16))) uint32_t stage_all[2 * 2 * St::WAVE_WORDS];
  const uint32_t total = slice_off[NB];
  const uint32_t lane = threadIdx.x & 63u;
  uint32_t* stage = stage_all + __builtin_amdgcn_readfirstlane(threadIdx.x >> 6) * (2 * St::WAVE_WORDS);
  const bool probe = clk != nullptr && blockIdx.x == 0 && __builtin_amdgcn_readfirstlane(threadIdx.x >> 6) == 0;
  const long long c0 = probe ? clock64() : 0, w0 = probe ? wall_clock64() : 0;
  for (;;) {
    uint32_t chunk = 0;
    if (lane == 0) chunk = atomicAdd(chunk_counter, 1u);
    chunk = __builtin_amdgcn_readfirstlane(chunk);
    if ((uint64_t)chunk * 64 >= total) {
      if (probe && lane == 0) {
        atomicAdd(clk, (unsigned long long)(clock64() - c0));
        atomicAdd(clk + 1, (unsigned long long)(wall_clock64() - w0));
      }
      if (clk != nullptr && lane == 0) {
        const unsigned long long now = (unsigned long long)wall_clock64();
        const uint32_t waves = gridDim.x * (blockDim.x >> 6);
        const uint32_t k = atomicAdd(chunk_counter + 1, 1u);
        atomicAdd(clk + CLK_ACC_EXIT_SUM, now);
        if (k == 0) {
          atomicAdd(clk + CLK_ACC_EXIT_FIRST, now);
          atomicAdd(clk + CLK_ACC_LAUNCHES, 1ull);
          atomicMax(clk + CLK_ACC_WAVES, (unsigned long long)waves);
        }
        if (k == waves - 1) atomicAdd(clk + CLK_ACC_EXIT_LAST, now);
      }
      break;
    }
    const uint32_t t = chunk * 64 + lane;
    if (t >= total) continue;
    uint32_t lo = chunk_rank[chunk], hi = min(lo + lane + 1u, NB);
    while (hi - lo > 1) {
      const uint32_t mid = (lo + hi) >> 1;
      if (slice_off[mid] <= t) lo = mid; else hi = mid;
    }
    const uint32_t r = lo;
    const uint32_t k = order[r];
    const uint32_t s = t - slice_off[r];
    const uint32_t ns = slice_off[r + 1] - slice_off[r];
    const uint32_t b0 = bstart[k];
    const uint32_t len = bstart[k + 1] - b0;
    uint32_t e = b0 + (uint32_t)(((uint64_t)s * len) / ns);
    const uint32_t e1 = b0 + (uint32_t)(((uint64_t)(s + 1) * len) / ns);
    const uint32_t dst = ns == 1 ? (k | 0x80000000u) : t;
    XYZZ<C> acc;
    acc.x = Fd::zero(); acc.y = Fd::zero(); acc.zz = Fd::one(); acc.zzz = Fd::one();
    bool finite = false;
    uint32_t v_cur = 0, v_next = 0;
    uint32_t it = 0;
    if (e < e1) {
      v_cur = vals[e];
      if (e + 1 < e1) v_next = vals[e + 1];
      St::issue(recs, v_cur & 0x7fffffffu, stage);
    }
    while (e < e1) {
      asm volatile("s_waitcnt vmcnt(0) lgkmcnt(0)" ::: "memory");
      const uint32_t* cur = stage + (it & 1u) * St::WAVE_WORDS;
      const uint32_t v = v_cur;
      ++e;
      ++it;
      if (e < e1) {
        v_cur = v_next;
        St::issue(recs, v_cur & 0x7fffffffu, stage + (it & 1u) * St::WAVE_WORDS);
        if (e + 1 < e1) v_next = vals[e + 1];
      }
      Fe<F> x, y;
      const uint32_t flag = St::read(cur, lane, x, y);
      if (flag & 1u) continue;
      if (!finite) {
        acc.x = x; acc.y = Fd::cneg_canonical(y, v >> 31);
        finite = true;
      } else {
        acc = Ec<C>::madd_finite(acc, x, y, (v >> 31) != 0, finite);
        if (!finite) { acc.zz = Fd::one(); acc.zzz = Fd::one(); }
      }
    }
    if (!finite) acc = Ec<C>::infinity();
    store_xyzz<C>((dst >> 31) ? buckets : partials, dst & 0x7fffffffu, acc);
  }
}

#ifndef KZG_SIDE_WAVES
#define KZG_SIDE_WAVES 3
#endif
#define KZG_SIDE_VGPRS __attribute__((amdgpu_waves_per_eu(KZG_SIDE_WAVES, KZG_SIDE_WAVES)))
#ifndef KZG_REDUCE_PRIO
#define KZG_REDUCE_PRIO 3
#endif

constexpr uint32_t HEAVY_RANKS = 256;
constexpr uint32_t HEAVY_NS = 64;

template <class C, int WB>
__global__ __launch_bounds__(256) KZG_SIDE_VGPRS void msm_finalize_heavy_kernel(const uint32_t* partials, const uint32_t* order,
                                                                 const uint32_t* slice_off, uint32_t* buckets) {
  __builtin_amdgcn_s_setprio(KZG_REDUCE_PRIO);
  constexpr int N = C::Fp::N;
  __shared__ __attribute__((aligned(16))) uint32_t xch[3 * 4 * N];
  const uint32_t r = blockIdx.x;
  const uint32_t p0 = slice_off[r], p1 = slice_off[r + 1];
  if (p1 - p0 <= HEAVY_NS) return;
  XYZZ<C> acc = Ec<C>::infinity();
  for (uint32_t p = p0 + threadIdx.x; p < p1; p += blockDim.x) acc = Ec<C>::add(acc, load_xyzz<C>(partials, p));
#pragma unroll
  for (int m = 1; m < 64; m <<= 1) acc = Ec<C>::add(acc, shfl_xor_xyzz<C>(acc, m));
  const uint32_t wave = threadIdx.x >> 6;
  if ((threadIdx.x & 63) == 0 && wave) store_xyzz<C>(xch, wave - 1, acc);
  __syncthreads();
  if (threadIdx.x == 0) {
    for (int k = 0; k < 3; ++k) acc = Ec<C>::add(acc, load_xyzz<C>(xch, k));
    store_xyzz<C>(buckets, order[r], acc);
  }
}

template <class C, int WB>
__global__ __launch_bounds__(128) KZG_SIDE_VGPRS void msm_finalize_kernel(const uint32_t* partials, const uint32_t* order,
                                                           const uint32_t* slice_off, uint32_t* buckets) {
  __builtin_amdgcn_s_setprio(KZG_REDUCE_PRIO);
  constexpr uint32_t FIN = Win<WB>::FIN, NB = Win<WB>::NB;
  static_assert(NB % (64 / FIN) == 0, "a wave covers whole ranks inside the bucket range");
  const uint32_t gt = blockIdx.x * blockDim.x + threadIdx.x;
  const uint32_t r = gt / FIN, g = gt % FIN;
  if (r >= NB) return;
  const uint32_t r_first = (gt & ~63u) / FIN, r_last = (gt | 63u) / FIN;
  if (slice_off[r_first + 1] - slice_off[r_first] == 1 && slice_off[r_last + 1] - slice_off[r_last] == 1) return;
  const uint32_t p0 = slice_off[r], p1 = slice_off[r + 1];
  const uint32_t cnt = p1 - p0;
  const bool mine = cnt != 1 && !(r < HEAVY_RANKS && cnt > HEAVY_NS);
  XYZZ<C> acc = Ec<C>::infinity();
  if (mine)
    for (uint32_t p = p0 + g; p < p1; p += FIN) acc = Ec<C>::add(acc, load_xyzz<C>(partials, p));
#pragma unroll
  for (int m = 1; m < (int)FIN; m <<= 1) acc = Ec<C>::add(acc, shfl_xor_xyzz<C>(acc, m));
  if (g == 0 && mine) store_xyzz<C>(buckets, order[r], acc);
}

constexpr uint32_t RC_CH = 8;
constexpr uint32_t RC_L2 = 16;

template <class C, int WB>
__global__ __launch_bounds__(128) KZG_SIDE_VGPRS void msm_rc1_kernel(const uint32_t* buckets, uint32_t* colpart,
                                                      uint32_t* rowpart) {
  __builtin_amdgcn_s_setprio(KZG_REDUCE_PRIO);
  constexpr int LO = Win<WB>::LO;
  constexpr uint32_t NCHR = (1u << LO) / RC_CH;
  const uint32_t L = blockIdx.x * blockDim.x + threadIdx.x;
  if (L >= Win<WB>::NB / RC_CH) return;
  XYZZ<C> acc = Ec<C>::infinity();
  if (blockIdx.y == 0) {
    const uint32_t lo = L & ((1u << LO) - 1), chunk = L >> LO;
    for (uint32_t e = 0; e < RC_CH; ++e) {
      const uint32_t v = ((chunk * RC_CH + e) << LO) + lo;
      if (v) acc = Ec<C>::add(acc, load_xyzz<C>(buckets, v - 1));
    }
    store_xyzz<C>(colpart, L, acc);
  } else {
    const uint32_t c = L & (NCHR - 1), hi = L / NCHR;
    for (uint32_t e = 0; e < RC_CH; ++e) {
      const uint32_t v = (hi << LO) + e * NCHR + c;
      if (v) acc = Ec<C>::add(acc, load_xyzz<C>(buckets, v - 1));
    }
    store_xyzz<C>(rowpart, L, acc);
  }
}

template <class C, int WB>
__global__ __launch_bounds__(128) KZG_SIDE_VGPRS void msm_rc2_kernel(const uint32_t* colpart, const uint32_t* rowpart,
                                                      uint32_t* colsum, uint32_t* rowsum) {
  __builtin_amdgcn_s_setprio(KZG_REDUCE_PRIO);
  constexpr int LO = Win<WB>::LO, HI = Win<WB>::HI;
  constexpr uint32_t NCHC = (1u << HI) / RC_CH, NCHR = (1u << LO) / RC_CH;
  const uint32_t gt = blockIdx.x * blockDim.x + threadIdx.x;
  const uint32_t vec = gt / RC_L2, g = gt % RC_L2;
  XYZZ<C> acc = Ec<C>::infinity();
  const bool is_col = vec < (1u << LO);
  const uint32_t row = vec - (1u << LO);
  if (is_col) {
    for (uint32_t q = g; q < NCHC; q += RC_L2) acc = Ec<C>::add(acc, load_xyzz<C>(colpart, (q << LO) + vec));
  } else if (row < (1u << HI)) {
    for (uint32_t q = g; q < NCHR; q += RC_L2) acc = Ec<C>::add(acc, load_xyzz<C>(rowpart, row * NCHR + q));
  }
#pragma unroll
  for (int m = 1; m < (int)RC_L2; m <<= 1) acc = Ec<C>::add(acc, shfl_xor_xyzz<C>(acc, m));
  if (g == 0) {
    if (is_col) store_xyzz<C>(colsum, vec, acc);
    else if (row < (1u << HI)) store_xyzz<C>(rowsum, row, acc);
  }
}

template <class C, int WB>
__global__ __launch_bounds__(128) KZG_SIDE_VGPRS void msm_planes_kernel(const uint32_t* rowsum, const uint32_t* colsum,
                                                         const uint32_t* buckets, uint32_t* out) {
  __builtin_amdgcn_s_setprio(KZG_REDUCE_PRIO);
  constexpr int LO = Win<WB>::LO, HI = Win<WB>::HI, N = C::Fp::N;
  __shared__ __attribute__((aligned(16))) uint32_t xch[4 * N];
  const uint32_t blk = blockIdx.x, tid = threadIdx.x;
  XYZZ<C> acc = Ec<C>::infinity();
  if (blk < (uint32_t)(HI + LO)) {
    const bool cols = blk >= (uint32_t)HI;
    const uint32_t b = cols ? blk - HI : blk;
    const uint32_t members = (cols ? (1u << LO) : (1u << HI)) >> 1;
    const uint32_t* src = cols ? colsum : rowsum;
    for (uint32_t q = tid; q < members; q += blockDim.x) {
      const uint32_t i = ((q >> b) << (b + 1)) | (1u << b) | (q & ((1u << b) - 1));
      acc = Ec<C>::add(acc, load_xyzz<C>(src, i));
    }
#pragma unroll
    for (int m = 1; m < 64; m <<= 1) acc = Ec<C>::add(acc, shfl_xor_xyzz<C>(acc, m));
    if (tid == 64) store_xyzz<C>(xch, 0, acc);
    __syncthreads();
    if (tid == 0) acc = Ec<C>::add(acc, load_xyzz<C>(xch, 0));
  } else {
    acc = load_xyzz<C>(buckets, Win<WB>::NB - 1);
  }
  if (tid == 0) store_xyzz<C>(out, blk, acc);
}

template <class C>
size_t rec_bytes() { return (size_t)C::REC_WORDS * 4; }

int pick_win_bits(size_t n) { return n >= (1u << 18) ? 20 : 16; }
int nwin_of(int wb) { return (256 + wb - 1) / wb; }

}


template <class C>
static int g1_import_t(Ctx* c, const uint32_t* d_xy, const uint8_t* d_inf, size_t n, bool range, uint32_t* d_recs,
                       uint32_t* d_bad) {
  const dim3 grid((uint32_t)((n + 255) / 256));
  if (range)
    hipLaunchKernelGGL((g1_import_kernel<C, true>), grid, dim3(256), 0, c->stream, d_xy, d_inf, d_recs, n, d_bad);
  else
    hipLaunchKernelGGL((g1_import_kernel<C, false>), grid, dim3(256), 0, c->stream, d_xy, d_inf, d_recs, n, d_bad);
  KZG_HIP(c, hipGetLastError());
  return KZG_OK;
}
int g1_import(Ctx* c, const uint32_t* d_xy, const uint8_t* d_inf, size_t n, bool range, uint32_t* d_recs,
              uint32_t* d_bad) {
  return KZG_BY_CURVE(c, g1_import_t, c, d_xy, d_inf, n, range, d_recs, d_bad);
}

template <class C>
static int srs_build_windows(Ctx* c, Srs* s) {
  const size_t n = s->n;
  const uint32_t blocks = (uint32_t)((n + 127) / 128);
  for (int j = 1; j < s->nwin; ++j) {
    hipLaunchKernelGGL(srs_window_kernel<C>, dim3(blocks), dim3(128), 0, c->stream,
                       s->recs + (size_t)(j - 1) * n * C::REC_WORDS, s->recs + (size_t)j * n * C::REC_WORDS, n,
                       s->win_bits);
    KZG_HIP(c, hipGetLastError());
  }
  KZG_HIP(c, hipStreamSynchronize(c->stream));
  return KZG_OK;
}

static int srs_alloc(Ctx* c, size_t n, size_t rec_bytes, const char* bad_size, SrsPtr* out) {
  if (n == 0 || n * (size_t)16 >= (1ull << 31)) return set_err(c, KZG_ERR_ARG, bad_size);
  SrsPtr s(new Srs());
  s->n = n;
  s->curve = c->curve;
  s->win_bits = pick_win_bits(n);
  s->nwin = nwin_of(s->win_bits);
  const hipError_t e = hipMalloc(reinterpret_cast<void**>(&s->recs), (size_t)s->nwin * n * rec_bytes);
  if (e != hipSuccess) return set_err(c, KZG_ERR_ALLOC, "hipMalloc(SRS table)", e);
  *out = std::move(s);
  return KZG_OK;
}

template <class C>
static int srs_load_device_t(Ctx* c, const uint32_t* d_xy, const uint8_t* d_inf, size_t n, Srs** out) {
  SrsPtr s;
  int rc = srs_alloc(c, n, rec_bytes<C>(), "kzg_srs_load_g1: bad size", &s);
  if (rc) return rc;
  DevTmp<uint32_t> d_bad;
  if (d_bad.alloc(4) != hipSuccess) return set_err(c, KZG_ERR_ALLOC, "hipMalloc");
  KZG_HIP(c, hipMemsetAsync(d_bad, 0, 4, c->stream));
  if ((rc = g1_import(c, d_xy, d_inf, n, false, s->recs, d_bad))) return rc;
  uint32_t bad = 0;
  KZG_HIP(c, hipMemcpyAsync(&bad, d_bad, 4, hipMemcpyDeviceToHost, c->stream));
  KZG_HIP(c, hipStreamSynchronize(c->stream));
  if (bad) return set_err(c, KZG_ERR_ARG, "kzg_srs_load_g1: point not on the curve");
  if ((rc = srs_build_windows<C>(c, s.get()))) return rc;
  *out = s.release();
  return KZG_OK;
}

template <class C>
static int srs_load_t(Ctx* c, const uint64_t* xy, const uint8_t* inf, size_t n, Srs** out) {
  using F = typename C::Fp;
  if (n == 0 || n * (size_t)16 >= (1ull << 31)) return set_err(c, KZG_ERR_ARG, "kzg_srs_load_g1: bad size");
  DevTmp<uint32_t> d_xy;
  DevTmp<uint8_t> d_inf;
  const size_t xy_bytes = n * 2 * F::NW * 4;
  if (d_xy.alloc(xy_bytes) != hipSuccess || (inf && d_inf.alloc(n) != hipSuccess))
    return set_err(c, KZG_ERR_ALLOC, "hipMalloc");
  KZG_HIP(c, hipMemcpyAsync(d_xy, xy, xy_bytes, hipMemcpyHostToDevice, c->stream));
  if (inf) KZG_HIP(c, hipMemcpyAsync(d_inf, inf, n, hipMemcpyHostToDevice, c->stream));
  return srs_load_device_t<C>(c, d_xy, d_inf, n, out);
}

static const uint64_t GEN_BN254[8] = {1, 0, 0, 0, 2, 0, 0, 0};
static const uint64_t GEN_BLS[12] = {
    0xfb3af00adb22c6bbull, 0x6c55e83ff97a1aefull, 0xa14e3a3f171bac58ull, 0xc3688c4f9774b905ull,
    0x2695638c4fa9ac0full, 0x17f1d3a73197d794ull,
    0x0caa232946c5e7e1ull, 0xd03cc744a2888ae4ull, 0x00db18cb2c04b3edull, 0xfcf5e095d5d00af6ull,
    0xa09e30ed741d8ae4ull, 0x08b3f481e3aaa0f1ull};

const uint64_t* g1_generator_limbs(int curve) { return curve == 0 ? GEN_BN254 : GEN_BLS; }

template <class C>
static int srs_generate_t(Ctx* c, const uint32_t* tau_words, size_t start, size_t n, Srs** out, size_t run_len,
                          size_t inner_stride, size_t outer_stride, const uint32_t* d_scalars = nullptr) {
  using F = typename C::Fp;
  using Fr = typename C::Fr;
  const uint64_t* gen_xy = C::ID == 0 ? GEN_BN254 : GEN_BLS;
  SrsPtr s;
  int rc = srs_alloc(c, n, rec_bytes<C>(), "kzg_srs_generate: bad size", &s);
  if (rc) return rc;
  DevTmp<uint32_t> d_g, d_tab, d_tau, d_xy, d_bad;
  if (d_g.alloc(rec_bytes<C>()) != hipSuccess || d_tab.alloc(32 * 255 * rec_bytes<C>()) != hipSuccess ||
      d_tau.alloc(Fr::N * 4) != hipSuccess || d_xy.alloc(2 * F::NW * 4) != hipSuccess || d_bad.alloc(4) != hipSuccess)
    return set_err(c, KZG_ERR_ALLOC, "hipMalloc");
  const Fe<Fr> tau = Field<Fr>::to_mont(Field<Fr>::from_words(tau_words));
  KZG_HIP(c, hipMemcpy(d_tau, tau.l, Fr::N * 4, hipMemcpyHostToDevice));
  KZG_HIP(c, hipMemcpy(d_xy, gen_xy, 2 * F::NW * 4, hipMemcpyHostToDevice));
  KZG_HIP(c, hipMemsetAsync(d_bad, 0, 4, c->stream));
  hipLaunchKernelGGL((g1_import_kernel<C, false>), dim3(1), dim3(64), 0, c->stream, d_xy.get(),
                     (const uint8_t*)nullptr, d_g.get(), (size_t)1, d_bad.get());
  hipLaunchKernelGGL(gen_table_kernel<C>, dim3(32), dim3(256), 0, c->stream, d_g.get(), d_tab.get());
  hipLaunchKernelGGL(srs_generate_kernel<C>, dim3((uint32_t)((n + 127) / 128)), dim3(128), 0, c->stream, d_tab.get(),
                     d_tau.get(), s->recs, start, n, run_len, inner_stride, outer_stride, d_scalars);
  KZG_HIP(c, hipGetLastError());
  KZG_HIP(c, hipStreamSynchronize(c->stream));
  if ((rc = srs_build_windows<C>(c, s.get()))) return rc;
  *out = s.release();
  return KZG_OK;
}

int srs_load(Ctx* c, const uint64_t* xy, const uint8_t* inf, size_t n, Srs** out) {
  return KZG_BY_CURVE(c, srs_load_t, c, xy, inf, n, out);
}
int srs_load_device(Ctx* c, const uint32_t* d_xy, const uint8_t* d_inf, size_t n, Srs** out) {
  return KZG_BY_CURVE(c, srs_load_device_t, c, d_xy, d_inf, n, out);
}
int srs_generate(Ctx* c, const uint64_t* tau, size_t start, size_t n, Srs** out, size_t run_len, size_t inner_stride,
                 size_t outer_stride) {
  const uint32_t* t = reinterpret_cast<const uint32_t*>(tau);
  if (run_len == 0) { run_len = n ? n : 1; inner_stride = 1; outer_stride = 0; }
  return KZG_BY_CURVE(c, srs_generate_t, c, t, start, n, out, run_len, inner_stride, outer_stride);
}
int srs_generate_scalars(Ctx* c, const uint32_t* d_scalars, size_t n, Srs** out) {
  static const uint32_t zero[8] = {0};
  return KZG_BY_CURVE(c, srs_generate_t, c, zero, 0, n, out, n ? n : 1, 1, 0, d_scalars);
}
int srs_create(Ctx* c, size_t n, SrsPtr* out) { return srs_alloc(c, n, srs_rec_bytes(c->curve), "SRS: bad size", out); }
int srs_finish_windows(Ctx* c, Srs* s) {
  return KZG_BY_CURVE(c, srs_build_windows, c, s);
}
void srs_window0_view(const Ctx* c, uint32_t* recs, size_t n, Srs* out) {
  *out = Srs();
  out->n = n;
  out->curve = c->curve;
  out->win_bits = pick_win_bits(n);
  out->nwin = 1;
  out->recs = recs;
}
size_t srs_rec_bytes(int curve) { return curve == 0 ? rec_bytes<Bn254>() : rec_bytes<Bls12_381>(); }
void srs_free(Srs* s) {
  if (!s) return;
  hipFree(s->recs);
  hipFree(s->d_wpow);
  delete s;
}

template <class C>
static int srs_export_t(Ctx* c, const Srs* s, size_t start, size_t count, uint64_t* xy, uint8_t* inf) {
  using F = typename C::Fp;
  if (start + count > s->n) return set_err(c, KZG_ERR_ARG, "kzg_srs_export: range");
  if (count == 0) return KZG_OK;
  DevTmp<uint32_t> d_xy;
  DevTmp<uint8_t> d_inf;
  KZG_HIP(c, d_xy.alloc(count * 2 * F::NW * 4));
  KZG_HIP(c, d_inf.alloc(count));
  hipLaunchKernelGGL(srs_export_kernel<C>, dim3((uint32_t)((count + 255) / 256)), dim3(256), 0, c->stream, s->recs,
                     start, count, d_xy.get(), d_inf.get());
  KZG_HIP(c, hipGetLastError());
  KZG_HIP(c, hipMemcpyAsync(xy, d_xy, count * 2 * F::NW * 4, hipMemcpyDeviceToHost, c->stream));
  KZG_HIP(c, hipMemcpyAsync(inf, d_inf, count, hipMemcpyDeviceToHost, c->stream));
  KZG_HIP(c, hipStreamSynchronize(c->stream));
  return KZG_OK;
}
int srs_export(Ctx* c, const Srs* s, size_t start, size_t count, uint64_t* xy, uint8_t* inf) {
  return KZG_BY_CURVE(c, srs_export_t, c, s, start, count, xy, inf);
}

constexpr int NSLOT = 4;
#ifndef KZG_PIPE_PRIO_A
#define KZG_PIPE_PRIO_A 1
#endif

struct MsmSlot {
  DevBuf prep_ws, vals, bstart, order, slice_off, counter, chunk_rank;
  DevBuf scal;
  DevBuf partials, buckets, rowsum, colsum, rowpart, colpart, tb;
  void* h_tb = nullptr;
  uint64_t* out_eval = nullptr;
  hipEvent_t ev_in = nullptr;
  hipEvent_t ev_p = nullptr;
  hipEvent_t ev_a = nullptr;
  hipEvent_t ev_b = nullptr;
  bool pending = false;
  int win_bits = 0;
  uint64_t* out_xy = nullptr;
  uint8_t* out_inf = nullptr;
};

struct MsmWork {
  MsmSlot slot[NSLOT];
  hipStream_t stream_s = nullptr, stream_a = nullptr;
  int deferred = -1;
  int next = 0;
  uint32_t acc_blocks = 0;
};

static MsmWork* get_work(Ctx* c) {
  if (!c->msm_work) c->msm_work = new MsmWork();
  return static_cast<MsmWork*>(c->msm_work);
}
bool msm_accumulate_in_flight(Ctx* c) {
  MsmWork* w = static_cast<MsmWork*>(c->msm_work);
  if (!w) return false;
  for (auto& sl : w->slot)
    if (sl.pending && sl.ev_a && hipEventQuery(sl.ev_a) == hipErrorNotReady) return true;
  (void)hipGetLastError();
  return false;
}

void msm_free_work(Ctx* c) {
  MsmWork* w = static_cast<MsmWork*>(c->msm_work);
  if (!w) return;
  for (auto& sl : w->slot) {
    for (DevBuf* b : {&sl.scal, &sl.prep_ws, &sl.vals, &sl.bstart, &sl.order, &sl.slice_off, &sl.counter, &sl.chunk_rank, &sl.partials,
                      &sl.buckets, &sl.rowsum, &sl.colsum, &sl.rowpart, &sl.colpart, &sl.tb})
      hipFree(b->p);
    if (sl.h_tb) hipHostFree(sl.h_tb);
    for (hipEvent_t e : {sl.ev_in, sl.ev_p, sl.ev_a, sl.ev_b})
      if (e) hipEventDestroy(e);
  }
  for (hipStream_t st : {w->stream_s, w->stream_a})
    if (st) hipStreamDestroy(st);
  delete w;
  c->msm_work = nullptr;
}

template <class C>
static int msm_queue_deferred(Ctx* c, MsmWork* w);

template <class C, int WB>
static int msm_enqueue(Ctx* c, const Srs* s, const uint32_t* d_scalars, uint32_t n, MsmWork* w, int slot_idx) {
  using W = Win<WB>;
  constexpr size_t PT = 4 * C::Fp::N * 4;
  constexpr uint32_t NB = W::NB;
  MsmSlot& sl = w->slot[slot_idx];
  const uint32_t m = n * W::NWIN;
  const uint32_t max_slices = m / W::SEG + NB + 1;
  int rc;
  if ((rc = ensure_buf(c, sl.prep_ws, msm_prep_workspace_bytes(n, WB)))) return rc;
  if ((rc = ensure_buf(c, sl.vals, (size_t)m * 4))) return rc;
  if ((rc = ensure_buf(c, sl.bstart, (size_t)(NB + 2) * 4))) return rc;
  if ((rc = ensure_buf(c, sl.order, (size_t)NB * 4))) return rc;
  if ((rc = ensure_buf(c, sl.slice_off, (size_t)(NB + 2) * 4))) return rc;
  if ((rc = ensure_buf(c, sl.partials, (size_t)max_slices * PT))) return rc;
  if ((rc = ensure_buf(c, sl.buckets, (size_t)NB * PT))) return rc;
  if ((rc = ensure_buf(c, sl.rowsum, ((size_t)1 << W::HI) * PT))) return rc;
  if ((rc = ensure_buf(c, sl.colsum, ((size_t)1 << W::LO) * PT))) return rc;
  if ((rc = ensure_buf(c, sl.rowpart, (size_t)(NB / RC_CH) * PT))) return rc;
  if ((rc = ensure_buf(c, sl.colpart, (size_t)(NB / RC_CH) * PT))) return rc;
  if ((rc = ensure_buf(c, sl.tb, (size_t)MAX_NPART * PT))) return rc;
  if ((rc = ensure_buf(c, sl.counter, 256))) return rc;
  const uint32_t nchunk_max = max_slices / 64 + 1;
  if ((rc = ensure_buf(c, sl.chunk_rank, (size_t)nchunk_max * 4))) return rc;
  if (!sl.h_tb) KZG_HIP(c, hipHostMalloc(&sl.h_tb, MAX_NPART * 4 * 16 * 4 + 32));
  for (hipEvent_t* e : {&sl.ev_in, &sl.ev_p, &sl.ev_a, &sl.ev_b})
    if (!*e) KZG_HIP(c, hipEventCreateWithFlags(e, hipEventDisableTiming));
  if (!w->stream_a) {
    int prio_least = 0, prio_greatest = 0;
    KZG_HIP(c, hipDeviceGetStreamPriorityRange(&prio_least, &prio_greatest));
    KZG_HIP(c, hipStreamCreateWithPriority(&w->stream_a, hipStreamNonBlocking, KZG_PIPE_PRIO_A ? prio_greatest : 0));
    KZG_HIP(c, hipStreamCreateWithFlags(&w->stream_s, hipStreamNonBlocking));
    int cus = 0;
    KZG_HIP(c, hipDeviceGetAttribute(&cus, hipDeviceAttributeMultiprocessorCount, c->device));
    const char* ew = getenv("KZG_ACC_WGS_PER_CU");
    const int per_cu = ew && atoi(ew) > 0 ? atoi(ew) : 4;
    w->acc_blocks = (uint32_t)std::max(cus, 1) * (uint32_t)per_cu;
  }
  sl.win_bits = WB;

  auto* vals = static_cast<uint32_t*>(sl.vals.p);
  auto* bstart = static_cast<uint32_t*>(sl.bstart.p);
  auto* order = static_cast<uint32_t*>(sl.order.p);
  auto* slice_off = static_cast<uint32_t*>(sl.slice_off.p);
  hipStream_t sp = w->stream_s, sa = w->stream_a;

  static const bool copy_scalars = [] { const char* e = getenv("KZG_COMMIT_COPY_SCALARS"); return !(e && atoi(e) == 0); }();
  if (copy_scalars) {
    if ((rc = ensure_buf(c, sl.scal, (size_t)n * 32))) return rc;
    KZG_HIP(c, hipMemcpyAsync(sl.scal.p, d_scalars, (size_t)n * 32, hipMemcpyDeviceToDevice, c->stream));
    d_scalars = static_cast<const uint32_t*>(sl.scal.p);
  }
  KZG_HIP(c, hipEventRecord(sl.ev_in, c->stream));
  KZG_HIP(c, hipStreamWaitEvent(sp, sl.ev_in, 0));
#ifdef KZG_TIMING_SKIP_PREP
  static int prep_runs = 0;
  if (prep_runs++ >= 2 * NSLOT) { KZG_HIP(c, hipMemsetAsync(sl.counter.p, 0, 8, sp)); } else
#endif
  if ((rc = msm_prep_enqueue(c, sp, WB, d_scalars, n, (uint32_t)s->n, W::SEG, sl.prep_ws.p, vals, bstart, order,
                             slice_off, static_cast<uint32_t*>(sl.counter.p),
                             static_cast<uint32_t*>(sl.chunk_rank.p), nchunk_max)))
    return rc;
  KZG_HIP(c, hipEventRecord(sl.ev_p, sp));
  if (!copy_scalars) KZG_HIP(c, hipStreamWaitEvent(c->stream, sl.ev_p, 0));
  if ((rc = msm_queue_deferred<C>(c, w))) return rc;

  KZG_HIP(c, hipStreamWaitEvent(sa, sl.ev_p, 0));
  {
    ProfScope ps(c, "msm_accumulate", sa);
    hipLaunchKernelGGL((msm_accumulate_kernel<C, WB>), dim3(std::min(w->acc_blocks, (max_slices + 127) / 128)),
                       dim3(128), 0, sa, s->recs, vals, bstart, order, slice_off,
                       static_cast<uint32_t*>(sl.partials.p), static_cast<uint32_t*>(sl.buckets.p),
                       static_cast<uint32_t*>(sl.counter.p), static_cast<const uint32_t*>(sl.chunk_rank.p),
                       c->prof_on ? c->clk_probe : nullptr);
  }
  KZG_HIP(c, hipGetLastError());
  KZG_HIP(c, hipEventRecord(sl.ev_a, sa));

  w->deferred = slot_idx;
  return KZG_OK;
}

template <class C, int WB>
static int msm_enqueue_reduce(Ctx* c, MsmWork* w, MsmSlot& sl) {
  using W = Win<WB>;
  constexpr size_t PT = 4 * C::Fp::N * 4;
  constexpr uint32_t NB = W::NB;
  auto* order = static_cast<uint32_t*>(sl.order.p);
  auto* slice_off = static_cast<uint32_t*>(sl.slice_off.p);
  hipStream_t sb = w->stream_s;
  KZG_HIP(c, hipStreamWaitEvent(sb, sl.ev_a, 0));
#ifndef KZG_TIMING_SKIP_REDUCE
  {
    ProfScope ps(c, "msm_finalize", sb);
    hipLaunchKernelGGL((msm_finalize_heavy_kernel<C, WB>), dim3(std::min<uint32_t>(HEAVY_RANKS, NB)), dim3(256), 0, sb,
                       static_cast<uint32_t*>(sl.partials.p), order, slice_off, static_cast<uint32_t*>(sl.buckets.p));
    hipLaunchKernelGGL((msm_finalize_kernel<C, WB>), dim3((uint32_t)(((uint64_t)NB * W::FIN + 127) / 128)), dim3(128),
                       0, sb, static_cast<uint32_t*>(sl.partials.p), order, slice_off,
                       static_cast<uint32_t*>(sl.buckets.p));
  }
  {
    ProfScope ps(c, "msm_reduce", sb);
    hipLaunchKernelGGL((msm_rc1_kernel<C, WB>), dim3((NB / RC_CH + 127) / 128, 2), dim3(128), 0, sb,
                       static_cast<uint32_t*>(sl.buckets.p), static_cast<uint32_t*>(sl.colpart.p),
                       static_cast<uint32_t*>(sl.rowpart.p));
    hipLaunchKernelGGL((msm_rc2_kernel<C, WB>), dim3((((1u << W::LO) + (1u << W::HI)) * RC_L2 + 127) / 128),
                       dim3(128), 0, sb, static_cast<uint32_t*>(sl.colpart.p), static_cast<uint32_t*>(sl.rowpart.p),
                       static_cast<uint32_t*>(sl.colsum.p), static_cast<uint32_t*>(sl.rowsum.p));
    hipLaunchKernelGGL((msm_planes_kernel<C, WB>), dim3(W::NPART), dim3(128), 0, sb,
                       static_cast<uint32_t*>(sl.rowsum.p), static_cast<uint32_t*>(sl.colsum.p),
                       static_cast<uint32_t*>(sl.buckets.p), static_cast<uint32_t*>(sl.tb.p));
  }
#endif
  KZG_HIP(c, hipGetLastError());
  KZG_HIP(c, hipMemcpyAsync(sl.h_tb, sl.tb.p, W::NPART * PT, hipMemcpyDeviceToHost, sb));
  KZG_HIP(c, hipEventRecord(sl.ev_b, sb));
  return KZG_OK;
}

template <class C>
static int msm_queue_deferred(Ctx* c, MsmWork* w) {
  if (w->deferred < 0) return KZG_OK;
  MsmSlot& sl = w->slot[w->deferred];
  w->deferred = -1;
  return sl.win_bits == 20 ? msm_enqueue_reduce<C, 20>(c, w, sl) : msm_enqueue_reduce<C, 16>(c, w, sl);
}

template <class C, int WB>
static void msm_finish_host(const void* h_tb, uint64_t* out_xy, uint8_t* out_inf) {
  using W = Win<WB>;
  constexpr int N = C::Fp::N;
  const uint32_t* p = static_cast<const uint32_t*>(h_tb);
  auto pt = [&](int idx) {
    XYZZ<C> t;
    memcpy(t.x.l, p + (size_t)idx * 4 * N, N * 4);
    memcpy(t.y.l, p + (size_t)idx * 4 * N + N, N * 4);
    memcpy(t.zz.l, p + (size_t)idx * 4 * N + 2 * N, N * 4);
    memcpy(t.zzz.l, p + (size_t)idx * 4 * N + 3 * N, N * 4);
    return t;
  };
  XYZZ<C> acc = pt(W::HI + W::LO);
  for (int e = W::HI + W::LO - 1; e >= 0; --e) {
    acc = Ec<C>::dbl(acc);
    if (e >= W::LO) acc = Ec<C>::add(acc, pt(e - W::LO));
    if (e < W::LO) acc = Ec<C>::add(acc, pt(W::HI + e));
  }
  *out_inf = affine_to_words<C>(Ec<C>::to_affine(acc), reinterpret_cast<uint32_t*>(out_xy));
}

template <class C>
static int msm_retire(Ctx* c, MsmSlot& sl) {
  if (!sl.pending) { sl.out_eval = nullptr; return KZG_OK; }
  MsmWork* w = get_work(c);
  if (w->deferred >= 0 && &w->slot[w->deferred] == &sl) {
    int rc = msm_queue_deferred<C>(c, w);
    if (rc) return rc;
  }
  KZG_HIP(c, hipEventSynchronize(sl.ev_b));
  if (sl.win_bits == 20) msm_finish_host<C, 20>(sl.h_tb, sl.out_xy, sl.out_inf);
  else msm_finish_host<C, 16>(sl.h_tb, sl.out_xy, sl.out_inf);
  if (sl.out_eval) {
    memcpy(sl.out_eval, static_cast<const char*>(sl.h_tb) + MAX_NPART * 4 * 16 * 4, 32);
    sl.out_eval = nullptr;
  }
  sl.pending = false;
  return KZG_OK;
}

template <class C>
static int commit_flush_t(Ctx* c) {
  MsmWork* w = get_work(c);
  int rc = msm_queue_deferred<C>(c, w);
  for (int k = 0; k < NSLOT; ++k) {
    MsmSlot& sl = w->slot[(w->next + k) % NSLOT];
    int r2 = msm_retire<C>(c, sl);
    if (rc == KZG_OK) rc = r2;
  }
  if (rc == KZG_OK) KZG_HIP(c, hipStreamSynchronize(c->stream));
  return rc;
}

template <class C>
static int commit_t(Ctx* c, const Srs* s, const uint32_t* d_scalars, const size_t* lens, size_t n_polys,
                    size_t stride, uint64_t* out_xy, uint8_t* out_inf, bool drain, const uint32_t* d_eval,
                    uint64_t* out_eval) {
  using F = typename C::Fp;
  MsmWork* w = get_work(c);
  for (size_t p = 0; p < n_polys; ++p) {
    if (lens[p] > s->n) return set_err(c, KZG_ERR_DEGREE, "polynomial longer than the commitment key");
    if (lens[p] > stride) return set_err(c, KZG_ERR_ARG, "kzg_commit: lens[p] > stride");
  }
  int rc = KZG_OK;
  for (size_t p = 0; p < n_polys && rc == KZG_OK; ++p) {
    uint64_t* o = out_xy + p * 2 * (F::NW / 2);
    if (lens[p] == 0) {
      memset(o, 0, 2 * F::NW * 4);
      out_inf[p] = 1;
      if (d_eval && out_eval) {
        if ((rc = KZG_HIP_RC(c, hipMemcpyAsync(out_eval, d_eval, 32, hipMemcpyDeviceToHost, c->stream)))) break;
        rc = KZG_HIP_RC(c, hipStreamSynchronize(c->stream));
      }
      continue;
    }
    const int si = w->next;
    MsmSlot& sl = w->slot[si];
    w->next = (w->next + 1) % NSLOT;
    if ((rc = msm_retire<C>(c, sl))) break;
    uint64_t* slot_eval = nullptr;
    if (d_eval && out_eval) {
      if (!sl.h_tb && (rc = KZG_HIP_RC(c, hipHostMalloc(&sl.h_tb, MAX_NPART * 4 * 16 * 4 + 32)))) break;
      if ((rc = KZG_HIP_RC(c, hipMemcpyAsync(static_cast<char*>(sl.h_tb) + MAX_NPART * 4 * 16 * 4, d_eval, 32,
                                             hipMemcpyDeviceToHost, c->stream))))
        break;
      slot_eval = out_eval;
    }
    const uint32_t* sc = d_scalars + p * stride * 8;
    rc = s->win_bits == 20 ? msm_enqueue<C, 20>(c, s, sc, (uint32_t)lens[p], w, si)
                           : msm_enqueue<C, 16>(c, s, sc, (uint32_t)lens[p], w, si);
    if (rc) break;
    sl.pending = true;
    sl.out_eval = slot_eval;
    sl.out_xy = o;
    sl.out_inf = out_inf + p;
  }
  if (drain || rc != KZG_OK) {
    int r2 = commit_flush_t<C>(c);
    if (rc == KZG_OK) rc = r2;
  }
  return rc;
}

int commit_flush(Ctx* c) { return KZG_BY_CURVE(c, commit_flush_t, c); }

int commit_device(Ctx* c, const Srs* s, const uint32_t* d_scalars, const size_t* lens, size_t n_polys,
                  size_t stride, uint64_t* out_xy, uint8_t* out_inf, bool drain, const uint32_t* d_eval,
                  uint64_t* out_eval) {
  if (s->curve != c->curve) return set_err(c, KZG_ERR_ARG, "SRS belongs to another curve");
  if (d_eval && n_polys != 1) return set_err(c, KZG_ERR_ARG, "an evaluation rides with exactly one polynomial");
  return KZG_BY_CURVE(c, commit_t, c, s, d_scalars, lens, n_polys, stride, out_xy, out_inf, drain, d_eval, out_eval);
}

}
```

### kzg_snark_amd/csrc/msm_prep.h

```cpp
#pragma once
#include "internal.h"

namespace kzg {

size_t msm_prep_workspace_bytes(uint32_t n, int win_bits);

int msm_prep_enqueue(Ctx* c, hipStream_t sp, int win_bits, const uint32_t* d_scalars, uint32_t n, uint32_t srs_n,
                     uint32_t seg, void* ws, uint32_t* vals, uint32_t* bstart, uint32_t* order, uint32_t* slice_off,
                     uint32_t* chunk_counter, uint32_t* chunk_rank, uint32_t nchunk_max);

}
```

### kzg_snark_amd/csrc/msm_prep.hip

```cpp
#include <cstring>
#include <string.h>
#include <algorithm>
#include "internal.h"
#include "msm_prep.h"

namespace kzg {
namespace {

template <int WB, int LOBV = 8>
struct PW {
  static constexpr int NWIN = (256 + WB - 1) / WB;
  static constexpr uint32_t NB = 1u << (WB - 1);
  static constexpr int LOB = LOBV;
  static constexpr uint32_t BPB = 1u << LOB;
  static constexpr uint32_t NBIN = NB >> LOB;
};
constexpr uint32_t TPB = 256;
#ifndef KZG_PREP_PRIO
#define KZG_PREP_PRIO 3
#endif
#ifndef KZG_PREP_CH1
#define KZG_PREP_CH1 4096
#endif
constexpr uint32_t CH1 = KZG_PREP_CH1;
#ifndef KZG_PREP_CH2
#define KZG_PREP_CH2 8192
#endif
constexpr uint32_t CH2 = KZG_PREP_CH2;
#ifndef KZG_PREP_STAGE_CAP
#define KZG_PREP_STAGE_CAP 7168
#endif
#ifndef KZG_PREP_SWEEPS
#define KZG_PREP_SWEEPS 2
#endif
constexpr uint32_t SWEEPS = KZG_PREP_SWEEPS;
constexpr uint32_t STAGE_CAP = KZG_PREP_STAGE_CAP;
constexpr uint32_t CHL = 2048;
constexpr uint32_t NCLS = 256;

__device__ __forceinline__ void side_priority() { __builtin_amdgcn_s_setprio(KZG_PREP_PRIO); }

template <int WB, class Fn>
__device__ __forceinline__ void for_each_digit(const uint32_t* scalars, uint32_t i, Fn&& f) {
  const uint4* sp = reinterpret_cast<const uint4*>(scalars + (size_t)i * 8);
  const uint4 lo4 = sp[0], hi4 = sp[1];
  const uint32_t w[9] = {lo4.x, lo4.y, lo4.z, lo4.w, hi4.x, hi4.y, hi4.z, hi4.w, 0u};
  uint32_t carry = 0;
#pragma unroll
  for (int j = 0; j < PW<WB>::NWIN; ++j) {
    const int bit = j * WB, k = bit >> 5, sh = bit & 31;
    const uint64_t two = ((uint64_t)w[k + 1] << 32) | w[k];
    uint32_t d = ((uint32_t)(two >> sh) & ((1u << WB) - 1)) + carry;
    uint32_t neg = 0;
    if (d > (1u << (WB - 1))) { d = (1u << WB) - d; neg = 1; carry = 1; } else { carry = 0; }
    if (d) f((uint32_t)j, d - 1, neg);
  }
}

__device__ __forceinline__ uint32_t block_inclusive_scan(uint32_t v, uint32_t* sh) {
  const uint32_t tid = threadIdx.x;
  sh[tid] = v;
  __syncthreads();
#pragma unroll
  for (uint32_t off = 1; off < TPB; off <<= 1) {
    const uint32_t t = tid >= off ? sh[tid - off] : 0u;
    __syncthreads();
    sh[tid] += t;
    __syncthreads();
  }
  return sh[tid];
}


template <int WB, int LOBV>
__global__ __launch_bounds__(TPB) void prep_count1_kernel(const uint32_t* scalars, uint32_t n, uint32_t nchunk,
                                                          uint32_t* hist1) {
  using P = PW<WB, LOBV>;
  side_priority();
  __shared__ uint32_t hist[P::NBIN];
  for (uint32_t b = threadIdx.x; b < P::NBIN; b += TPB) hist[b] = 0;
  __syncthreads();
  const uint32_t base = blockIdx.x * CH1;
  for (uint32_t it = 0; it < CH1 / TPB; ++it) {
    const uint32_t i = base + it * TPB + threadIdx.x;
    if (i < n) for_each_digit<WB>(scalars, i, [&](uint32_t, uint32_t key, uint32_t) { atomicAdd(&hist[key >> P::LOB], 1u); });
  }
  __syncthreads();
  for (uint32_t b = threadIdx.x; b < P::NBIN; b += TPB) hist1[(size_t)b * nchunk + blockIdx.x] = hist[b];
}

__global__ __launch_bounds__(TPB) void prep_row_scan_kernel(uint32_t* hist, uint32_t len, uint32_t* row_total) {
  side_priority();
  __shared__ uint32_t sh[TPB];
  uint32_t* row = hist + (size_t)blockIdx.x * len;
  uint32_t carry = 0;
  for (uint32_t base = 0; base < len; base += TPB) {
    const uint32_t idx = base + threadIdx.x;
    const uint32_t v = idx < len ? row[idx] : 0u;
    const uint32_t incl = block_inclusive_scan(v, sh);
    if (idx < len) row[idx] = carry + incl - v;
    carry += sh[TPB - 1];
    __syncthreads();
  }
  if (threadIdx.x == 0) row_total[blockIdx.x] = carry;
}

template <int WB, int LOBV>
__global__ __launch_bounds__(TPB) void prep_bins_kernel(const uint32_t* bin_total, uint32_t* bin_start,
                                                        uint32_t* chunk_base, uint32_t* seg_of_chunk,
                                                        uint32_t* nchunk2, uint32_t* bstart_top) {
  using P = PW<WB, LOBV>;
  side_priority();
  __shared__ uint32_t sh[TPB];
  uint32_t size_carry = 0, chunk_carry = 0;
  for (uint32_t base = 0; base < P::NBIN; base += TPB) {
    const uint32_t s = base + threadIdx.x;
    const uint32_t size = s < P::NBIN ? bin_total[s] : 0u;
    const uint32_t nc = size > STAGE_CAP ? (size + CH2 - 1) / CH2 : 0u;
    const uint32_t size_incl = block_inclusive_scan(size, sh);
    const uint32_t size_tot = sh[TPB - 1];
    __syncthreads();
    const uint32_t nc_incl = block_inclusive_scan(nc, sh);
    const uint32_t nc_tot = sh[TPB - 1];
    __syncthreads();
    if (s < P::NBIN) {
      bin_start[s] = size_carry + size_incl - size;
      const uint32_t c0 = chunk_carry + nc_incl - nc;
      chunk_base[s] = c0;
      for (uint32_t q = 0; q < nc; ++q) seg_of_chunk[c0 + q] = s;
    }
    size_carry += size_tot;
    chunk_carry += nc_tot;
  }
  if (threadIdx.x == 0) {
    bin_start[P::NBIN] = size_carry;
    chunk_base[P::NBIN] = chunk_carry;
    *nchunk2 = chunk_carry;
    *bstart_top = size_carry;
  }
}

#ifndef KZG_PREP_PAIR
#define KZG_PREP_PAIR 0
#endif
__device__ __forceinline__ void store_pair(uint64_t* p, unsigned long long a, unsigned long long b) {
  typedef uint32_t u32x4 __attribute__((ext_vector_type(4), aligned(8)));
  u32x4 v = {(uint32_t)a, (uint32_t)(a >> 32), (uint32_t)b, (uint32_t)(b >> 32)};
  *reinterpret_cast<u32x4*>(p) = v;
}
template <int WB, int LOBV>
__global__ __launch_bounds__(TPB) void prep_scatter1_kernel(const uint32_t* scalars, uint32_t n, uint32_t srs_n,
                                                            uint32_t nchunk, const uint32_t* hist1,
                                                            const uint32_t* bin_start, uint64_t* ent) {
  using P = PW<WB, LOBV>;
  constexpr bool PAIR = KZG_PREP_PAIR && P::NBIN <= 2048;
  constexpr unsigned long long EMPTY = ~0ull;
  side_priority();
  __shared__ uint32_t cur[P::NBIN];
  __shared__ unsigned long long slot[PAIR ? P::NBIN : 1];
  const uint32_t chunk = blockIdx.x;
  for (uint32_t b = threadIdx.x; b < P::NBIN; b += TPB) {
    cur[b] = bin_start[b] + hist1[(size_t)b * nchunk + chunk];
    if (PAIR) slot[b] = EMPTY;
  }
  __syncthreads();
  const uint32_t base = chunk * CH1;
  for (uint32_t sweep = 0; sweep < SWEEPS; ++sweep) {
    const uint32_t b_lo = sweep * (P::NBIN / SWEEPS), b_hi = b_lo + P::NBIN / SWEEPS;
    for (uint32_t it = 0; it < CH1 / TPB; ++it) {
      const uint32_t i = base + it * TPB + threadIdx.x;
      if (i < n)
        for_each_digit<WB>(scalars, i, [&](uint32_t j, uint32_t key, uint32_t neg) {
          const uint32_t bin = key >> P::LOB;
          if (SWEEPS > 1 && (bin < b_lo || bin >= b_hi)) return;
          const unsigned long long mine =
              ((unsigned long long)(key & (P::BPB - 1)) << 32) | (unsigned long long)((j * srs_n + i) | (neg << 31));
          if constexpr (PAIR) {
            for (;;) {
              const unsigned long long seen = atomicCAS(&slot[bin], EMPTY, mine);
              if (seen == EMPTY) break;
              if (atomicCAS(&slot[bin], seen, EMPTY) == seen) {
                const uint32_t pos = atomicAdd(&cur[bin], 2u);
                store_pair(ent + pos, seen, mine);
                break;
              }
            }
          } else {
            const uint32_t pos = atomicAdd(&cur[bin], 1u);
            ent[pos] = mine;
          }
        });
    }
    if constexpr (PAIR) {
      __syncthreads();
      for (uint32_t b = b_lo + threadIdx.x; b < b_hi; b += TPB) {
        const unsigned long long e = slot[b];
        if (e != EMPTY) {
          ent[atomicAdd(&cur[b], 1u)] = e;
          slot[b] = EMPTY;
        }
      }
      __syncthreads();
    }
  }
}


struct Chunk2 {
  uint32_t seg, e0, e1;
};
__device__ __forceinline__ Chunk2 chunk2_of(uint32_t g, const uint32_t* bin_start, const uint32_t* chunk_base,
                                            const uint32_t* seg_of_chunk) {
  Chunk2 c;
  c.seg = seg_of_chunk[g];
  const uint32_t lc = g - chunk_base[c.seg];
  c.e0 = bin_start[c.seg] + lc * CH2;
  c.e1 = min(c.e0 + CH2, bin_start[c.seg + 1]);
  return c;
}

template <int WB, int LOBV>
__global__ __launch_bounds__(TPB) void prep_count2_kernel(const uint64_t* ent, const uint32_t* bin_start,
                                                          const uint32_t* chunk_base, const uint32_t* seg_of_chunk,
                                                          const uint32_t* nchunk2, uint32_t* hist2) {
  using P = PW<WB, LOBV>;
  side_priority();
  const uint32_t g = blockIdx.x;
  if (g >= *nchunk2) return;
  __shared__ uint32_t hist[P::BPB];
  for (uint32_t b = threadIdx.x; b < P::BPB; b += TPB) hist[b] = 0;
  __syncthreads();
  const Chunk2 c = chunk2_of(g, bin_start, chunk_base, seg_of_chunk);
  for (uint32_t e = c.e0 + threadIdx.x; e < c.e1; e += TPB) atomicAdd(&hist[(uint32_t)(ent[e] >> 32)], 1u);
  __syncthreads();
  for (uint32_t b = threadIdx.x; b < P::BPB; b += TPB) hist2[(size_t)g * P::BPB + b] = hist[b];
}

template <int WB, int LOBV>
__global__ __launch_bounds__(TPB) void prep_scan2_kernel(uint32_t* hist2, const uint32_t* bin_start,
                                                         const uint32_t* chunk_base, uint32_t* bstart) {
  using P = PW<WB, LOBV>;
  constexpr uint32_t PER = P::BPB >= TPB ? P::BPB / TPB : 1;
  side_priority();
  __shared__ uint32_t tot[P::BPB];
  __shared__ uint32_t sh[TPB];
  const uint32_t s = blockIdx.x;
  const uint32_t c0 = chunk_base[s], c1 = chunk_base[s + 1];
  if (c0 == c1) return;
  for (uint32_t b = threadIdx.x; b < P::BPB; b += TPB) {
    uint32_t run = 0;
    for (uint32_t c = c0; c < c1; ++c) {
      const uint32_t v = hist2[(size_t)c * P::BPB + b];
      hist2[(size_t)c * P::BPB + b] = run;
      run += v;
    }
    tot[b] = run;
  }
  __syncthreads();
  const bool own = threadIdx.x * PER < P::BPB;
  uint32_t mine = 0;
#pragma unroll
  for (uint32_t q = 0; q < PER; ++q) mine += own ? tot[threadIdx.x * PER + q] : 0u;
  const uint32_t incl = block_inclusive_scan(mine, sh);
  uint32_t run = bin_start[s] + incl - mine;
  if (own) {
#pragma unroll
    for (uint32_t q = 0; q < PER; ++q) {
      bstart[(size_t)s * P::BPB + threadIdx.x * PER + q] = run;
      run += tot[threadIdx.x * PER + q];
    }
  }
}

template <int WB, int LOBV>
__global__ __launch_bounds__(TPB) void prep_scatter2_kernel(const uint64_t* ent, const uint32_t* bin_start,
                                                            const uint32_t* chunk_base, const uint32_t* seg_of_chunk,
                                                            const uint32_t* nchunk2, const uint32_t* hist2,
                                                            const uint32_t* bstart, uint32_t* vals) {
  using P = PW<WB, LOBV>;
  side_priority();
  const uint32_t g = blockIdx.x;
  if (g >= *nchunk2) return;
  __shared__ uint32_t cur[P::BPB];
  const Chunk2 c = chunk2_of(g, bin_start, chunk_base, seg_of_chunk);
  for (uint32_t b = threadIdx.x; b < P::BPB; b += TPB)
    cur[b] = bstart[(size_t)c.seg * P::BPB + b] + hist2[(size_t)g * P::BPB + b];
  __syncthreads();
  for (uint32_t e = c.e0 + threadIdx.x; e < c.e1; e += TPB) {
    const uint64_t v = ent[e];
    const uint32_t pos = atomicAdd(&cur[(uint32_t)(v >> 32)], 1u);
    vals[pos] = (uint32_t)v;
  }
}

template <int WB, int LOBV>
__global__ __launch_bounds__(TPB) void prep_binsort_kernel(const uint64_t* ent, const uint32_t* bin_start,
                                                           uint32_t* bstart, uint32_t* vals) {
  using P = PW<WB, LOBV>;
  constexpr uint32_t PER = P::BPB >= TPB ? P::BPB / TPB : 1;
  constexpr uint32_t EPT = STAGE_CAP / TPB;
  static_assert(STAGE_CAP % TPB == 0, "the stage is a whole number of entries per thread");
  side_priority();
  __shared__ uint32_t cur[P::BPB];
  __shared__ uint32_t sh[TPB];
  __shared__ uint32_t stage[STAGE_CAP];
  const uint32_t s = blockIdx.x;
  const uint32_t e0 = bin_start[s], e1 = bin_start[s + 1];
  const uint32_t size = e1 - e0;
  if (size > STAGE_CAP) return;
  for (uint32_t b = threadIdx.x; b < P::BPB; b += TPB) cur[b] = 0;
  uint64_t mine_e[EPT];
#pragma unroll
  for (uint32_t q = 0; q < EPT; ++q) {
    const uint32_t e = e0 + q * TPB + threadIdx.x;
    mine_e[q] = e < e1 ? ent[e] : ~0ull;
  }
  __syncthreads();
#pragma unroll
  for (uint32_t q = 0; q < EPT; ++q)
    if ((uint32_t)(mine_e[q] >> 32) < P::BPB) atomicAdd(&cur[(uint32_t)(mine_e[q] >> 32)], 1u);
  __syncthreads();
  const bool own = threadIdx.x * PER < P::BPB;
  uint32_t mine = 0;
#pragma unroll
  for (uint32_t q = 0; q < PER; ++q) mine += own ? cur[threadIdx.x * PER + q] : 0u;
  const uint32_t incl = block_inclusive_scan(mine, sh);
  uint32_t run = incl - mine;
  if (own) {
#pragma unroll
    for (uint32_t q = 0; q < PER; ++q) {
      const uint32_t cnt = cur[threadIdx.x * PER + q];
      bstart[(size_t)s * P::BPB + threadIdx.x * PER + q] = e0 + run;
      cur[threadIdx.x * PER + q] = run;
      run += cnt;
    }
  }
  __syncthreads();
#pragma unroll
  for (uint32_t q = 0; q < EPT; ++q)
    if ((uint32_t)(mine_e[q] >> 32) < P::BPB) stage[atomicAdd(&cur[(uint32_t)(mine_e[q] >> 32)], 1u)] = (uint32_t)mine_e[q];
  __syncthreads();
  for (uint32_t i = threadIdx.x; i < size; i += TPB) vals[e0 + i] = stage[i];
}


__device__ __forceinline__ uint32_t length_class(uint32_t len) { return 255u - min(len, 255u); }

template <int WB>
__global__ __launch_bounds__(TPB) void prep_lcount_kernel(const uint32_t* bstart, uint32_t nchunk, uint32_t* histl) {
  using P = PW<WB>;
  side_priority();
  __shared__ uint32_t hist[NCLS];
  hist[threadIdx.x] = 0;
  __syncthreads();
  const uint32_t base = blockIdx.x * CHL;
  for (uint32_t it = 0; it < CHL / TPB; ++it) {
    const uint32_t k = base + it * TPB + threadIdx.x;
    if (k < P::NB) atomicAdd(&hist[length_class(bstart[k + 1] - bstart[k])], 1u);
  }
  __syncthreads();
  histl[(size_t)threadIdx.x * nchunk + blockIdx.x] = hist[threadIdx.x];
}

__global__ __launch_bounds__(TPB) void prep_classes_kernel(const uint32_t* class_total, uint32_t* class_start) {
  side_priority();
  __shared__ uint32_t sh[TPB];
  const uint32_t v = class_total[threadIdx.x];
  const uint32_t incl = block_inclusive_scan(v, sh);
  class_start[threadIdx.x] = incl - v;
}

template <int WB>
__global__ __launch_bounds__(TPB) void prep_lscatter_kernel(const uint32_t* bstart, uint32_t nchunk,
                                                            const uint32_t* histl, const uint32_t* class_start,
                                                            uint32_t* order) {
  using P = PW<WB>;
  side_priority();
  __shared__ uint32_t cur[NCLS];
  cur[threadIdx.x] = class_start[threadIdx.x] + histl[(size_t)threadIdx.x * nchunk + blockIdx.x];
  __syncthreads();
  const uint32_t base = blockIdx.x * CHL;
  for (uint32_t it = 0; it < CHL / TPB; ++it) {
    const uint32_t k = base + it * TPB + threadIdx.x;
    if (k < P::NB) order[atomicAdd(&cur[length_class(bstart[k + 1] - bstart[k])], 1u)] = k;
  }
}

template <int WB>
__device__ __forceinline__ uint32_t slices_of_rank(const uint32_t* bstart, const uint32_t* order, uint32_t seg, uint32_t r) {
  if (r >= PW<WB>::NB) return 0u;
  const uint32_t k = order[r];
  return (bstart[k + 1] - bstart[k] + seg - 1) / seg;
}
template <int WB>
__global__ __launch_bounds__(TPB) void prep_ns_totals_kernel(const uint32_t* bstart, const uint32_t* order, uint32_t seg,
                                                             uint32_t* blk_total) {
  side_priority();
  __shared__ uint32_t sh[TPB];
  const uint32_t v = slices_of_rank<WB>(bstart, order, seg, blockIdx.x * TPB + threadIdx.x);
  block_inclusive_scan(v, sh);
  if (threadIdx.x == 0) blk_total[blockIdx.x] = sh[TPB - 1];
}
template <int WB>
__global__ __launch_bounds__(TPB) void prep_slice_off_kernel(const uint32_t* bstart, const uint32_t* order, uint32_t seg,
                                                             const uint32_t* blk_prefix, uint32_t* slice_off,
                                                             uint32_t* chunk_counter) {
  side_priority();
  __shared__ uint32_t sh[TPB];
  const uint32_t r = blockIdx.x * TPB + threadIdx.x;
  const uint32_t v = slices_of_rank<WB>(bstart, order, seg, r);
  const uint32_t incl = block_inclusive_scan(v, sh);
  if (r <= PW<WB>::NB) slice_off[r] = blk_prefix[blockIdx.x] + incl - v;
  if (r == 0) { chunk_counter[0] = 0; chunk_counter[1] = 0; }
}

template <int WB>
__global__ __launch_bounds__(TPB) void prep_chunk_rank_kernel(const uint32_t* slice_off, uint32_t nchunk_max,
                                                              uint32_t* chunk_rank) {
  constexpr uint32_t NB = PW<WB>::NB;
  side_priority();
  const uint32_t c = blockIdx.x * TPB + threadIdx.x;
  if (c >= nchunk_max) return;
  const uint32_t t = c * 64u;
  uint32_t lo = 0, hi = NB;
  if (t < slice_off[NB]) {
    while (hi - lo > 1) {
      const uint32_t mid = (lo + hi) >> 1;
      if (slice_off[mid] <= t) lo = mid; else hi = mid;
    }
  }
  chunk_rank[c] = lo;
}

size_t align256(size_t x) { return (x + 255) & ~(size_t)255; }

template <int WB, int LOBV>
struct Layout {
  using P = PW<WB, LOBV>;
  uint32_t m, nchunk1, nchunk2_max, nchunkl;
  size_t off_ent, off_hist1, off_bin_total, off_bin_start, off_chunk_base, off_seg_of_chunk, off_nchunk2, off_hist2,
      off_histl, off_class_total, off_class_start, off_ns, total;
  explicit Layout(uint32_t n) {
    m = n * (uint32_t)P::NWIN;
    nchunk1 = (n + CH1 - 1) / CH1;
    nchunk2_max = m / CH2 + P::NBIN + 1;
    nchunkl = (P::NB + CHL - 1) / CHL;
    size_t t = 0;
    auto take = [&](size_t bytes) { const size_t o = t; t += align256(bytes); return o; };
    off_ent = take((size_t)m * 8);
    off_hist1 = take((size_t)P::NBIN * nchunk1 * 4);
    off_bin_total = take((size_t)P::NBIN * 4);
    off_bin_start = take((size_t)(P::NBIN + 1) * 4);
    off_chunk_base = take((size_t)(P::NBIN + 1) * 4);
    off_seg_of_chunk = take((size_t)nchunk2_max * 4);
    off_nchunk2 = take(4);
    off_hist2 = take((size_t)nchunk2_max * P::BPB * 4);
    off_histl = take((size_t)NCLS * nchunkl * 4);
    off_class_total = take(NCLS * 4);
    off_class_start = take(NCLS * 4);
    off_ns = take((size_t)((P::NB + 1 + TPB - 1) / TPB + 2) * 4);
    total = t;
  }
};

template <int WB, int LOBV>
int prep_enqueue_t(Ctx* c, hipStream_t sp, const uint32_t* d_scalars, uint32_t n, uint32_t srs_n, uint32_t seg,
                   void* ws, uint32_t* vals, uint32_t* bstart, uint32_t* order, uint32_t* slice_off,
                   uint32_t* chunk_counter, uint32_t* chunk_rank, uint32_t nchunk_max) {
  using P = PW<WB, LOBV>;
  const Layout<WB, LOBV> L(n);
  char* w = static_cast<char*>(ws);
  auto* ent = reinterpret_cast<uint64_t*>(w + L.off_ent);
  auto* hist1 = reinterpret_cast<uint32_t*>(w + L.off_hist1);
  auto* bin_total = reinterpret_cast<uint32_t*>(w + L.off_bin_total);
  auto* bin_start = reinterpret_cast<uint32_t*>(w + L.off_bin_start);
  auto* chunk_base = reinterpret_cast<uint32_t*>(w + L.off_chunk_base);
  auto* seg_of_chunk = reinterpret_cast<uint32_t*>(w + L.off_seg_of_chunk);
  auto* nchunk2 = reinterpret_cast<uint32_t*>(w + L.off_nchunk2);
  auto* hist2 = reinterpret_cast<uint32_t*>(w + L.off_hist2);
  auto* histl = reinterpret_cast<uint32_t*>(w + L.off_histl);
  auto* class_total = reinterpret_cast<uint32_t*>(w + L.off_class_total);
  auto* class_start = reinterpret_cast<uint32_t*>(w + L.off_class_start);
  auto* ns = reinterpret_cast<uint32_t*>(w + L.off_ns);
  {
    ProfScope ps(c, "msm_partition1", sp);
    hipLaunchKernelGGL((prep_count1_kernel<WB, LOBV>), dim3(L.nchunk1), dim3(TPB), 0, sp, d_scalars, n, L.nchunk1, hist1);
    hipLaunchKernelGGL(prep_row_scan_kernel, dim3(P::NBIN), dim3(TPB), 0, sp, hist1, L.nchunk1, bin_total);
    hipLaunchKernelGGL((prep_bins_kernel<WB, LOBV>), dim3(1), dim3(TPB), 0, sp, bin_total, bin_start, chunk_base, seg_of_chunk,
                       nchunk2, bstart + P::NB);
    hipLaunchKernelGGL((prep_scatter1_kernel<WB, LOBV>), dim3(L.nchunk1), dim3(TPB), 0, sp, d_scalars, n, srs_n, L.nchunk1,
                       hist1, bin_start, ent);
  }
  KZG_HIP(c, hipGetLastError());
  {
    ProfScope ps(c, "msm_partition2", sp);
    hipLaunchKernelGGL((prep_binsort_kernel<WB, LOBV>), dim3(P::NBIN), dim3(TPB), 0, sp, ent, bin_start, bstart, vals);
    hipLaunchKernelGGL((prep_count2_kernel<WB, LOBV>), dim3(L.nchunk2_max), dim3(TPB), 0, sp, ent, bin_start, chunk_base,
                       seg_of_chunk, nchunk2, hist2);
    hipLaunchKernelGGL((prep_scan2_kernel<WB, LOBV>), dim3(P::NBIN), dim3(TPB), 0, sp, hist2, bin_start, chunk_base, bstart);
    hipLaunchKernelGGL((prep_scatter2_kernel<WB, LOBV>), dim3(L.nchunk2_max), dim3(TPB), 0, sp, ent, bin_start, chunk_base,
                       seg_of_chunk, nchunk2, hist2, bstart, vals);
  }
  KZG_HIP(c, hipGetLastError());
  {
    ProfScope ps(c, "msm_order", sp);
    hipLaunchKernelGGL(prep_lcount_kernel<WB>, dim3(L.nchunkl), dim3(TPB), 0, sp, bstart, L.nchunkl, histl);
    hipLaunchKernelGGL(prep_row_scan_kernel, dim3(NCLS), dim3(TPB), 0, sp, histl, L.nchunkl, class_total);
    hipLaunchKernelGGL(prep_classes_kernel, dim3(1), dim3(TPB), 0, sp, class_total, class_start);
    hipLaunchKernelGGL(prep_lscatter_kernel<WB>, dim3(L.nchunkl), dim3(TPB), 0, sp, bstart, L.nchunkl, histl,
                       class_start, order);
    const uint32_t nblk = (P::NB + 1 + TPB - 1) / TPB;
    hipLaunchKernelGGL(prep_ns_totals_kernel<WB>, dim3(nblk), dim3(TPB), 0, sp, bstart, order, seg, ns);
    hipLaunchKernelGGL(prep_row_scan_kernel, dim3(1), dim3(TPB), 0, sp, ns, nblk, ns + nblk);
    hipLaunchKernelGGL(prep_slice_off_kernel<WB>, dim3(nblk), dim3(TPB), 0, sp, bstart, order, seg, ns, slice_off,
                       chunk_counter);
    hipLaunchKernelGGL(prep_chunk_rank_kernel<WB>, dim3((nchunk_max + TPB - 1) / TPB), dim3(TPB), 0, sp, slice_off,
                       nchunk_max, chunk_rank);
  }
  KZG_HIP(c, hipGetLastError());
  return KZG_OK;
}

}

static int lob_for(uint32_t n, int win_bits) {
  if (win_bits != 20) return 8;
  const uint64_t m = (uint64_t)n * PW<20>::NWIN;
  for (int lob = 8; lob > 6; --lob)
    if (m / (PW<20>::NB >> lob) + 4 * 82 <= STAGE_CAP) return lob;
  return 6;
}

size_t msm_prep_workspace_bytes(uint32_t n, int win_bits) {
  if (win_bits != 20) return Layout<16, 8>(n).total;
  switch (lob_for(n, win_bits)) {
    case 8: return Layout<20, 8>(n).total;
    case 7: return Layout<20, 7>(n).total;
    default: return Layout<20, 6>(n).total;
  }
}

int msm_prep_enqueue(Ctx* c, hipStream_t sp, int win_bits, const uint32_t* d_scalars, uint32_t n, uint32_t srs_n,
                     uint32_t seg, void* ws, uint32_t* vals, uint32_t* bstart, uint32_t* order, uint32_t* slice_off,
                     uint32_t* chunk_counter, uint32_t* chunk_rank, uint32_t nchunk_max) {
#define KZG_PREP_GO(WBV, LOBV) prep_enqueue_t<WBV, LOBV>(c, sp, d_scalars, n, srs_n, seg, ws, vals, bstart, order, slice_off, \
                                                        chunk_counter, chunk_rank, nchunk_max)
  if (win_bits != 20) return KZG_PREP_GO(16, 8);
  switch (lob_for(n, win_bits)) {
    case 8: return KZG_PREP_GO(20, 8);
    case 7: return KZG_PREP_GO(20, 7);
    default: return KZG_PREP_GO(20, 6);
  }
#undef KZG_PREP_GO
}

}
```

Baseline: 481.6 commits/s.

## Batch MSM accumulate and reduce across multiple polynomials in joint kernel launches

When earlier commits are still in flight, up to four polynomials are grouped. Each gets its own bucket prep, and then a joint work list merges their chunks, sorted by length class across all polys. A single accumulate kernel walks that list using per-poly descriptors, and the reduce kernels take a descriptor array indexed by blockIdx.z, so a group needs one launch chain instead of one per poly. This is meant to fill the GPU better and reduce tail imbalance and launch overhead. In exchange it adds extra prep kernels, more slot memory and indirection through descriptors.

```diff
diff --git a/kzg_snark_amd/csrc/api.hip b/kzg_snark_amd/csrc/api.hip
--- a/kzg_snark_amd/csrc/api.hip
+++ b/kzg_snark_amd/csrc/api.hip
@@ -33,7 +33,7 @@
   return code;
 }
 
-ProfScope::ProfScope(Ctx* ctx, const char* name, hipStream_t stream) : c(ctx) {
+ProfScope::ProfScope(Ctx* ctx, const char* name, hipStream_t stream, uint32_t parts_) : c(ctx), parts(parts_) {
   if (!c->prof_on) return;
   st = stream ? stream : c->stream;
   for (auto& sp : c->prof)
@@ -49,7 +49,7 @@
 ProfScope::~ProfScope() {
   if (!span) return;
   hipEventRecord(e1, st);
-  span->pending.emplace_back(e0, e1);
+  span->pending.push_back(ProfSpan::Pair{e0, e1, parts});
 }
 
 int ensure_buf(Ctx* c, DevBuf& b, size_t bytes) {
@@ -1015,7 +1015,7 @@
     if (sp.name != name) continue;
     for (auto& pr : sp.pending) {
       float ms = 0;
-      if (hipEventElapsedTime(&ms, pr.first, pr.second) == hipSuccess) { sp.total_ms += ms; sp.count += 1; }
+      if (hipEventElapsedTime(&ms, pr.first, pr.second) == hipSuccess) { sp.total_ms += ms; sp.count += pr.parts; }
       hipEventDestroy(pr.first);
       hipEventDestroy(pr.second);
     }
diff --git a/kzg_snark_amd/csrc/internal.h b/kzg_snark_amd/csrc/internal.h
--- a/kzg_snark_amd/csrc/internal.h
+++ b/kzg_snark_amd/csrc/internal.h
@@ -32,7 +32,8 @@
 
 struct ProfSpan {
   std::string name;
-  std::vector<std::pair<hipEvent_t, hipEvent_t>> pending;
+  struct Pair { hipEvent_t first, second; uint32_t parts; };
+  std::vector<Pair> pending;
   double total_ms = 0;
   uint64_t count = 0;
 };
@@ -108,7 +109,8 @@
   ProfSpan* span = nullptr;
   hipEvent_t e0 = nullptr, e1 = nullptr;
   hipStream_t st = nullptr;
-  ProfScope(Ctx* ctx, const char* name, hipStream_t stream = nullptr);
+  uint32_t parts = 1;
+  ProfScope(Ctx* ctx, const char* name, hipStream_t stream = nullptr, uint32_t parts = 1);
   ~ProfScope();
 };
 
diff --git a/kzg_snark_amd/csrc/msm.hip b/kzg_snark_amd/csrc/msm.hip
--- a/kzg_snark_amd/csrc/msm.hip
+++ b/kzg_snark_amd/csrc/msm.hip
@@ -215,7 +215,14 @@
   }
 };
 
-template <class C, int WB>
+__device__ __forceinline__ uint32_t uniform_word(uint32_t v) { return __builtin_amdgcn_readfirstlane(v); }
+template <class T>
+__device__ __forceinline__ T* uniform_ptr(T* const* slot) {
+  const uint32_t* w = reinterpret_cast<const uint32_t*>(slot);
+  const uint64_t v = (uint64_t)uniform_word(w[0]) | ((uint64_t)uniform_word(w[1]) << 32);
+  return reinterpret_cast<T*>(v);
+}
+template <class C, int WB, bool JOINT>
 __global__ __launch_bounds__(128, 3) void msm_accumulate_kernel(const uint32_t* recs, const uint32_t* vals,
                                                              const uint32_t* bstart, const uint32_t* order,
                                                              const uint32_t* slice_off, uint32_t* partials,
@@ -226,7 +233,9 @@
   using St = RecStage<C>;
   constexpr uint32_t NB = Win<WB>::NB;
   __shared__ __attribute__((aligned(16))) uint32_t stage_all[2 * 2 * St::WAVE_WORDS];
-  const uint32_t total = slice_off[NB];
+  const uint32_t* joint = vals;
+  uint32_t total = JOINT ? 0u : slice_off[NB];
+  const uint32_t work_end = JOINT ? joint[2] : 0u;
   const uint32_t lane = threadIdx.x & 63u;
   uint32_t* stage = stage_all + __builtin_amdgcn_readfirstlane(threadIdx.x >> 6) * (2 * St::WAVE_WORDS);
   const bool probe = clk != nullptr && blockIdx.x == 0 && __builtin_amdgcn_readfirstlane(threadIdx.x >> 6) == 0;
@@ -235,7 +244,7 @@
     uint32_t chunk = 0;
     if (lane == 0) chunk = atomicAdd(chunk_counter, 1u);
     chunk = __builtin_amdgcn_readfirstlane(chunk);
-    if ((uint64_t)chunk * 64 >= total) {
+    if (JOINT ? chunk >= work_end : (uint64_t)chunk * 64 >= total) {
       if (probe && lane == 0) {
         atomicAdd(clk, (unsigned long long)(clock64() - c0));
         atomicAdd(clk + 1, (unsigned long long)(wall_clock64() - w0));
@@ -253,6 +262,20 @@
         if (k == waves - 1) atomicAdd(clk + CLK_ACC_EXIT_LAST, now);
       }
       break;
+    }
+    if constexpr (JOINT) {
+      const uint32_t ent = uniform_word(joint[MSM_JOINT_LIST_OFF / 4 + chunk]);
+      const MsmPolyDesc* d = reinterpret_cast<const MsmPolyDesc*>(joint + MSM_JOINT_DESC_OFF / 4) +
+                             (ent >> MSM_JOINT_POLY_SHIFT);
+      chunk = ent & ((1u << MSM_JOINT_POLY_SHIFT) - 1);
+      vals = uniform_ptr(&d->vals);
+      bstart = uniform_ptr(&d->bstart);
+      order = uniform_ptr(&d->order);
+      slice_off = uniform_ptr(&d->slice_off);
+      chunk_rank = uniform_ptr(&d->chunk_rank);
+      partials = uniform_ptr(&d->partials);
+      buckets = uniform_ptr(&d->buckets);
+      total = uniform_word(d->total);
     }
     const uint32_t t = chunk * 64 + lane;
     if (t >= total) continue;
@@ -315,13 +338,30 @@
 #define KZG_REDUCE_PRIO 3
 #endif
 
+struct MsmReduceDesc {
+  const uint32_t *partials, *order, *slice_off;
+  uint32_t *buckets, *colpart, *rowpart, *colsum, *rowsum, *tb;
+};
+struct MsmReduceArgs {
+  MsmReduceDesc d[MSM_JOINT_MAX];
+};
+__device__ __forceinline__ MsmReduceDesc reduce_desc(const MsmReduceArgs& a) {
+  MsmReduceDesc d = a.d[0];
+#pragma unroll
+  for (int k = 1; k < MSM_JOINT_MAX; ++k)
+    if (blockIdx.z == (uint32_t)k) d = a.d[k];
+  return d;
+}
+
 constexpr uint32_t HEAVY_RANKS = 256;
 constexpr uint32_t HEAVY_NS = 64;
 
 template <class C, int WB>
-__global__ __launch_bounds__(256) KZG_SIDE_VGPRS void msm_finalize_heavy_kernel(const uint32_t* partials, const uint32_t* order,
-                                                                 const uint32_t* slice_off, uint32_t* buckets) {
+__global__ __launch_bounds__(256) KZG_SIDE_VGPRS void msm_finalize_heavy_kernel(MsmReduceArgs args) {
   __builtin_amdgcn_s_setprio(KZG_REDUCE_PRIO);
+  const MsmReduceDesc dsc = reduce_desc(args);
+  const uint32_t *partials = dsc.partials, *order = dsc.order, *slice_off = dsc.slice_off;
+  uint32_t* buckets = dsc.buckets;
   constexpr int N = C::Fp::N;
   __shared__ __attribute__((aligned(16))) uint32_t xch[3 * 4 * N];
   const uint32_t r = blockIdx.x;
@@ -341,9 +381,11 @@
 }
 
 template <class C, int WB>
-__global__ __launch_bounds__(128) KZG_SIDE_VGPRS void msm_finalize_kernel(const uint32_t* partials, const uint32_t* order,
-                                                           const uint32_t* slice_off, uint32_t* buckets) {
+__global__ __launch_bounds__(128) KZG_SIDE_VGPRS void msm_finalize_kernel(MsmReduceArgs args) {
   __builtin_amdgcn_s_setprio(KZG_REDUCE_PRIO);
+  const MsmReduceDesc dsc = reduce_desc(args);
+  const uint32_t *partials = dsc.partials, *order = dsc.order, *slice_off = dsc.slice_off;
+  uint32_t* buckets = dsc.buckets;
   constexpr uint32_t FIN = Win<WB>::FIN, NB = Win<WB>::NB;
   static_assert(NB % (64 / FIN) == 0, "a wave covers whole ranks inside the bucket range");
   const uint32_t gt = blockIdx.x * blockDim.x + threadIdx.x;
@@ -366,9 +408,11 @@
 constexpr uint32_t RC_L2 = 16;
 
 template <class C, int WB>
-__global__ __launch_bounds__(128) KZG_SIDE_VGPRS void msm_rc1_kernel(const uint32_t* buckets, uint32_t* colpart,
-                                                      uint32_t* rowpart) {
+__global__ __launch_bounds__(128) KZG_SIDE_VGPRS void msm_rc1_kernel(MsmReduceArgs args) {
   __builtin_amdgcn_s_setprio(KZG_REDUCE_PRIO);
+  const MsmReduceDesc dsc = reduce_desc(args);
+  const uint32_t* buckets = dsc.buckets;
+  uint32_t *colpart = dsc.colpart, *rowpart = dsc.rowpart;
   constexpr int LO = Win<WB>::LO;
   constexpr uint32_t NCHR = (1u << LO) / RC_CH;
   const uint32_t L = blockIdx.x * blockDim.x + threadIdx.x;
@@ -392,9 +436,11 @@
 }
 
 template <class C, int WB>
-__global__ __launch_bounds__(128) KZG_SIDE_VGPRS void msm_rc2_kernel(const uint32_t* colpart, const uint32_t* rowpart,
-                                                      uint32_t* colsum, uint32_t* rowsum) {
+__global__ __launch_bounds__(128) KZG_SIDE_VGPRS void msm_rc2_kernel(MsmReduceArgs args) {
   __builtin_amdgcn_s_setprio(KZG_REDUCE_PRIO);
+  const MsmReduceDesc dsc = reduce_desc(args);
+  const uint32_t *colpart = dsc.colpart, *rowpart = dsc.rowpart;
+  uint32_t *colsum = dsc.colsum, *rowsum = dsc.rowsum;
   constexpr int LO = Win<WB>::LO, HI = Win<WB>::HI;
   constexpr uint32_t NCHC = (1u << HI) / RC_CH, NCHR = (1u << LO) / RC_CH;
   const uint32_t gt = blockIdx.x * blockDim.x + threadIdx.x;
@@ -416,9 +462,11 @@
 }
 
 template <class C, int WB>
-__global__ __launch_bounds__(128) KZG_SIDE_VGPRS void msm_planes_kernel(const uint32_t* rowsum, const uint32_t* colsum,
-                                                         const uint32_t* buckets, uint32_t* out) {
+__global__ __launch_bounds__(128) KZG_SIDE_VGPRS void msm_planes_kernel(MsmReduceArgs args) {
   __builtin_amdgcn_s_setprio(KZG_REDUCE_PRIO);
+  const MsmReduceDesc dsc = reduce_desc(args);
+  const uint32_t *rowsum = dsc.rowsum, *colsum = dsc.colsum, *buckets = dsc.buckets;
+  uint32_t* out = dsc.tb;
   constexpr int LO = Win<WB>::LO, HI = Win<WB>::HI, N = C::Fp::N;
   __shared__ __attribute__((aligned(16))) uint32_t xch[4 * N];
   const uint32_t blk = blockIdx.x, tid = threadIdx.x;
@@ -623,6 +671,8 @@
 }
 
 constexpr int NSLOT = 4;
+constexpr int NSLOT_JOINT = 2 * MSM_JOINT_MAX;
+constexpr int NSLOT_ALL = NSLOT + NSLOT_JOINT;
 #ifndef KZG_PIPE_PRIO_A
 #define KZG_PIPE_PRIO_A 1
 #endif
@@ -644,10 +694,14 @@
 };
 
 struct MsmWork {
-  MsmSlot slot[NSLOT];
+  MsmSlot slot[NSLOT_ALL];
   hipStream_t stream_s = nullptr, stream_a = nullptr;
-  int deferred = -1;
-  int next = 0;
+  int deferred[MSM_JOINT_MAX] = {0};
+  int n_deferred = 0;
+  int next = 0, jnext = 0;
+  DevBuf joint[2];
+  hipEvent_t ev_j[2] = {nullptr, nullptr};
+  int joint_next = 0;
   uint32_t acc_blocks = 0;
 };
 
@@ -675,6 +729,10 @@
     for (hipEvent_t e : {sl.ev_in, sl.ev_p, sl.ev_a, sl.ev_b})
       if (e) hipEventDestroy(e);
   }
+  for (int k = 0; k < 2; ++k) {
+    hipFree(w->joint[k].p);
+    if (w->ev_j[k]) hipEventDestroy(w->ev_j[k]);
+  }
   for (hipStream_t st : {w->stream_s, w->stream_a})
     if (st) hipStreamDestroy(st);
   delete w;
@@ -684,14 +742,19 @@
 template <class C>
 static int msm_queue_deferred(Ctx* c, MsmWork* w);
 
+template <int WB>
+static uint32_t max_slices_of(uint32_t n) { return n * (uint32_t)Win<WB>::NWIN / Win<WB>::SEG + Win<WB>::NB + 1; }
+template <int WB>
+static uint32_t nchunk_max_of(uint32_t n) { return max_slices_of<WB>(n) / 64 + 1; }
+
 template <class C, int WB>
-static int msm_enqueue(Ctx* c, const Srs* s, const uint32_t* d_scalars, uint32_t n, MsmWork* w, int slot_idx) {
+static int msm_enqueue_prep(Ctx* c, const Srs* s, const uint32_t* d_scalars, uint32_t n, MsmWork* w, int slot_idx) {
   using W = Win<WB>;
   constexpr size_t PT = 4 * C::Fp::N * 4;
   constexpr uint32_t NB = W::NB;
   MsmSlot& sl = w->slot[slot_idx];
   const uint32_t m = n * W::NWIN;
-  const uint32_t max_slices = m / W::SEG + NB + 1;
+  const uint32_t max_slices = max_slices_of<WB>(n);
   int rc;
   if ((rc = ensure_buf(c, sl.prep_ws, msm_prep_workspace_bytes(n, WB)))) return rc;
   if ((rc = ensure_buf(c, sl.vals, (size_t)m * 4))) return rc;
@@ -706,7 +769,7 @@
   if ((rc = ensure_buf(c, sl.colpart, (size_t)(NB / RC_CH) * PT))) return rc;
   if ((rc = ensure_buf(c, sl.tb, (size_t)MAX_NPART * PT))) return rc;
   if ((rc = ensure_buf(c, sl.counter, 256))) return rc;
-  const uint32_t nchunk_max = max_slices / 64 + 1;
+  const uint32_t nchunk_max = nchunk_max_of<WB>(n);
   if ((rc = ensure_buf(c, sl.chunk_rank, (size_t)nchunk_max * 4))) return rc;
   if (!sl.h_tb) KZG_HIP(c, hipHostMalloc(&sl.h_tb, MAX_NPART * 4 * 16 * 4 + 32));
   for (hipEvent_t* e : {&sl.ev_in, &sl.ev_p, &sl.ev_a, &sl.ev_b})
@@ -728,7 +791,7 @@
   auto* bstart = static_cast<uint32_t*>(sl.bstart.p);
   auto* order = static_cast<uint32_t*>(sl.order.p);
   auto* slice_off = static_cast<uint32_t*>(sl.slice_off.p);
-  hipStream_t sp = w->stream_s, sa = w->stream_a;
+  hipStream_t sp = w->stream_s;
 
   static const bool copy_scalars = [] { const char* e = getenv("KZG_COMMIT_COPY_SCALARS"); return !(e && atoi(e) == 0); }();
   if (copy_scalars) {
@@ -740,7 +803,7 @@
   KZG_HIP(c, hipStreamWaitEvent(sp, sl.ev_in, 0));
 #ifdef KZG_TIMING_SKIP_PREP
   static int prep_runs = 0;
-  if (prep_runs++ >= 2 * NSLOT) { KZG_HIP(c, hipMemsetAsync(sl.counter.p, 0, 8, sp)); } else
+  if (prep_runs++ >= 2 * NSLOT_ALL) { KZG_HIP(c, hipMemsetAsync(sl.counter.p, 0, 8, sp)); } else
 #endif
   if ((rc = msm_prep_enqueue(c, sp, WB, d_scalars, n, (uint32_t)s->n, W::SEG, sl.prep_ws.p, vals, bstart, order,
                              slice_off, static_cast<uint32_t*>(sl.counter.p),
@@ -748,13 +811,25 @@
     return rc;
   KZG_HIP(c, hipEventRecord(sl.ev_p, sp));
   if (!copy_scalars) KZG_HIP(c, hipStreamWaitEvent(c->stream, sl.ev_p, 0));
+  return KZG_OK;
+}
+
+template <class C, int WB>
+static int msm_enqueue(Ctx* c, const Srs* s, const uint32_t* d_scalars, uint32_t n, MsmWork* w, int slot_idx) {
+  int rc;
+  if ((rc = msm_enqueue_prep<C, WB>(c, s, d_scalars, n, w, slot_idx))) return rc;
+  MsmSlot& sl = w->slot[slot_idx];
+  const uint32_t max_slices = max_slices_of<WB>(n);
+  hipStream_t sa = w->stream_a;
   if ((rc = msm_queue_deferred<C>(c, w))) return rc;
 
   KZG_HIP(c, hipStreamWaitEvent(sa, sl.ev_p, 0));
   {
     ProfScope ps(c, "msm_accumulate", sa);
-    hipLaunchKernelGGL((msm_accumulate_kernel<C, WB>), dim3(std::min(w->acc_blocks, (max_slices + 127) / 128)),
-                       dim3(128), 0, sa, s->recs, vals, bstart, order, slice_off,
+    hipLaunchKernelGGL((msm_accumulate_kernel<C, WB, false>), dim3(std::min(w->acc_blocks, (max_slices + 127) / 128)),
+                       dim3(128), 0, sa, s->recs, static_cast<const uint32_t*>(sl.vals.p),
+                       static_cast<const uint32_t*>(sl.bstart.p), static_cast<const uint32_t*>(sl.order.p),
+                       static_cast<const uint32_t*>(sl.slice_off.p),
                        static_cast<uint32_t*>(sl.partials.p), static_cast<uint32_t*>(sl.buckets.p),
                        static_cast<uint32_t*>(sl.counter.p), static_cast<const uint32_t*>(sl.chunk_rank.p),
                        c->prof_on ? c->clk_probe : nullptr);
@@ -762,53 +837,111 @@
   KZG_HIP(c, hipGetLastError());
   KZG_HIP(c, hipEventRecord(sl.ev_a, sa));
 
-  w->deferred = slot_idx;
+  w->deferred[0] = slot_idx;
+  w->n_deferred = 1;
   return KZG_OK;
 }
 
 template <class C, int WB>
-static int msm_enqueue_reduce(Ctx* c, MsmWork* w, MsmSlot& sl) {
+static int msm_enqueue_joint(Ctx* c, const Srs* s, MsmWork* w, const int* slots, const uint32_t* ns, int b) {
+  int rc;
+  MsmJointArgs a;
+  memset(&a, 0, sizeof(a));
+  uint32_t nchunk_max = 0, max_slices = 0;
+  for (int j = 0; j < b; ++j) {
+    const MsmSlot& sl = w->slot[slots[j]];
+    MsmPolyDesc& d = a.d[j];
+    d.vals = static_cast<const uint32_t*>(sl.vals.p);
+    d.bstart = static_cast<const uint32_t*>(sl.bstart.p);
+    d.order = static_cast<const uint32_t*>(sl.order.p);
+    d.slice_off = static_cast<const uint32_t*>(sl.slice_off.p);
+    d.chunk_rank = static_cast<const uint32_t*>(sl.chunk_rank.p);
+    d.partials = static_cast<uint32_t*>(sl.partials.p);
+    d.buckets = static_cast<uint32_t*>(sl.buckets.p);
+    nchunk_max = std::max(nchunk_max, nchunk_max_of<WB>(ns[j]));
+    max_slices += max_slices_of<WB>(ns[j]);
+  }
+  const int k = w->joint_next;
+  w->joint_next ^= 1;
+  if ((rc = ensure_buf(c, w->joint[k], msm_joint_bytes(nchunk_max, MSM_JOINT_MAX)))) return rc;
+  if (!w->ev_j[k]) KZG_HIP(c, hipEventCreateWithFlags(&w->ev_j[k], hipEventDisableTiming));
+  hipStream_t sp = w->stream_s, sa = w->stream_a;
+  if ((rc = msm_joint_enqueue(c, sp, WB, a, (uint32_t)b, nchunk_max, w->joint[k].p))) return rc;
+  KZG_HIP(c, hipEventRecord(w->ev_j[k], sp));
+  if ((rc = msm_queue_deferred<C>(c, w))) return rc;
+
+  KZG_HIP(c, hipStreamWaitEvent(sa, w->ev_j[k], 0));
+  {
+    ProfScope ps(c, "msm_accumulate", sa, (uint32_t)b);
+    auto* joint = static_cast<uint32_t*>(w->joint[k].p);
+    hipLaunchKernelGGL((msm_accumulate_kernel<C, WB, true>), dim3(std::min(w->acc_blocks, (max_slices + 127) / 128)),
+                       dim3(128), 0, sa, s->recs, joint, nullptr, nullptr, nullptr, nullptr, nullptr, joint, nullptr,
+                       c->prof_on ? c->clk_probe : nullptr);
+  }
+  KZG_HIP(c, hipGetLastError());
+  for (int j = 0; j < b; ++j) {
+    KZG_HIP(c, hipEventRecord(w->slot[slots[j]].ev_a, sa));
+    w->deferred[j] = slots[j];
+  }
+  w->n_deferred = b;
+  return KZG_OK;
+}
+
+template <class C, int WB>
+static int msm_enqueue_reduce(Ctx* c, MsmWork* w, const int* slots, int nb) {
   using W = Win<WB>;
   constexpr size_t PT = 4 * C::Fp::N * 4;
   constexpr uint32_t NB = W::NB;
-  auto* order = static_cast<uint32_t*>(sl.order.p);
-  auto* slice_off = static_cast<uint32_t*>(sl.slice_off.p);
   hipStream_t sb = w->stream_s;
-  KZG_HIP(c, hipStreamWaitEvent(sb, sl.ev_a, 0));
+  MsmReduceArgs a;
+  memset(&a, 0, sizeof(a));
+  for (int j = 0; j < nb; ++j) {
+    MsmSlot& sl = w->slot[slots[j]];
+    KZG_HIP(c, hipStreamWaitEvent(sb, sl.ev_a, 0));
+    MsmReduceDesc& d = a.d[j];
+    d.partials = static_cast<const uint32_t*>(sl.partials.p);
+    d.order = static_cast<const uint32_t*>(sl.order.p);
+    d.slice_off = static_cast<const uint32_t*>(sl.slice_off.p);
+    d.buckets = static_cast<uint32_t*>(sl.buckets.p);
+    d.colpart = static_cast<uint32_t*>(sl.colpart.p);
+    d.rowpart = static_cast<uint32_t*>(sl.rowpart.p);
+    d.colsum = static_cast<uint32_t*>(sl.colsum.p);
+    d.rowsum = static_cast<uint32_t*>(sl.rowsum.p);
+    d.tb = static_cast<uint32_t*>(sl.tb.p);
+  }
+  const uint32_t z = (uint32_t)nb;
 #ifndef KZG_TIMING_SKIP_REDUCE
   {
-    ProfScope ps(c, "msm_finalize", sb);
-    hipLaunchKernelGGL((msm_finalize_heavy_kernel<C, WB>), dim3(std::min<uint32_t>(HEAVY_RANKS, NB)), dim3(256), 0, sb,
-                       static_cast<uint32_t*>(sl.partials.p), order, slice_off, static_cast<uint32_t*>(sl.buckets.p));
-    hipLaunchKernelGGL((msm_finalize_kernel<C, WB>), dim3((uint32_t)(((uint64_t)NB * W::FIN + 127) / 128)), dim3(128),
-                       0, sb, static_cast<uint32_t*>(sl.partials.p), order, slice_off,
-                       static_cast<uint32_t*>(sl.buckets.p));
+    ProfScope ps(c, "msm_finalize", sb, z);
+    hipLaunchKernelGGL((msm_finalize_heavy_kernel<C, WB>), dim3(std::min<uint32_t>(HEAVY_RANKS, NB), 1, z), dim3(256), 0,
+                       sb, a);
+    hipLaunchKernelGGL((msm_finalize_kernel<C, WB>), dim3((uint32_t)(((uint64_t)NB * W::FIN + 127) / 128), 1, z),
+                       dim3(128), 0, sb, a);
   }
   {
-    ProfScope ps(c, "msm_reduce", sb);
-    hipLaunchKernelGGL((msm_rc1_kernel<C, WB>), dim3((NB / RC_CH + 127) / 128, 2), dim3(128), 0, sb,
-                       static_cast<uint32_t*>(sl.buckets.p), static_cast<uint32_t*>(sl.colpart.p),
-                       static_cast<uint32_t*>(sl.rowpart.p));
-    hipLaunchKernelGGL((msm_rc2_kernel<C, WB>), dim3((((1u << W::LO) + (1u << W::HI)) * RC_L2 + 127) / 128),
-                       dim3(128), 0, sb, static_cast<uint32_t*>(sl.colpart.p), static_cast<uint32_t*>(sl.rowpart.p),
-                       static_cast<uint32_t*>(sl.colsum.p), static_cast<uint32_t*>(sl.rowsum.p));
-    hipLaunchKernelGGL((msm_planes_kernel<C, WB>), dim3(W::NPART), dim3(128), 0, sb,
-                       static_cast<uint32_t*>(sl.rowsum.p), static_cast<uint32_t*>(sl.colsum.p),
-                       static_cast<uint32_t*>(sl.buckets.p), static_cast<uint32_t*>(sl.tb.p));
+    ProfScope ps(c, "msm_reduce", sb, z);
+    hipLaunchKernelGGL((msm_rc1_kernel<C, WB>), dim3((NB / RC_CH + 127) / 128, 2, z), dim3(128), 0, sb, a);
+    hipLaunchKernelGGL((msm_rc2_kernel<C, WB>), dim3((((1u << W::LO) + (1u << W::HI)) * RC_L2 + 127) / 128, 1, z),
+                       dim3(128), 0, sb, a);
+    hipLaunchKernelGGL((msm_planes_kernel<C, WB>), dim3(W::NPART, 1, z), dim3(128), 0, sb, a);
   }
 #endif
   KZG_HIP(c, hipGetLastError());
-  KZG_HIP(c, hipMemcpyAsync(sl.h_tb, sl.tb.p, W::NPART * PT, hipMemcpyDeviceToHost, sb));
-  KZG_HIP(c, hipEventRecord(sl.ev_b, sb));
+  for (int j = 0; j < nb; ++j) {
+    MsmSlot& sl = w->slot[slots[j]];
+    KZG_HIP(c, hipMemcpyAsync(sl.h_tb, sl.tb.p, W::NPART * PT, hipMemcpyDeviceToHost, sb));
+    KZG_HIP(c, hipEventRecord(sl.ev_b, sb));
+  }
   return KZG_OK;
 }
 
 template <class C>
 static int msm_queue_deferred(Ctx* c, MsmWork* w) {
-  if (w->deferred < 0) return KZG_OK;
-  MsmSlot& sl = w->slot[w->deferred];
-  w->deferred = -1;
-  return sl.win_bits == 20 ? msm_enqueue_reduce<C, 20>(c, w, sl) : msm_enqueue_reduce<C, 16>(c, w, sl);
+  const int nd = w->n_deferred;
+  if (nd == 0) return KZG_OK;
+  w->n_deferred = 0;
+  return w->slot[w->deferred[0]].win_bits == 20 ? msm_enqueue_reduce<C, 20>(c, w, w->deferred, nd)
+                                                : msm_enqueue_reduce<C, 16>(c, w, w->deferred, nd);
 }
 
 template <class C, int WB>
@@ -837,10 +970,12 @@
 static int msm_retire(Ctx* c, MsmSlot& sl) {
   if (!sl.pending) { sl.out_eval = nullptr; return KZG_OK; }
   MsmWork* w = get_work(c);
-  if (w->deferred >= 0 && &w->slot[w->deferred] == &sl) {
-    int rc = msm_queue_deferred<C>(c, w);
-    if (rc) return rc;
-  }
+  for (int j = 0; j < w->n_deferred; ++j)
+    if (&w->slot[w->deferred[j]] == &sl) {
+      int rc = msm_queue_deferred<C>(c, w);
+      if (rc) return rc;
+      break;
+    }
   KZG_HIP(c, hipEventSynchronize(sl.ev_b));
   if (sl.win_bits == 20) msm_finish_host<C, 20>(sl.h_tb, sl.out_xy, sl.out_inf);
   else msm_finish_host<C, 16>(sl.h_tb, sl.out_xy, sl.out_inf);
@@ -856,8 +991,8 @@
 static int commit_flush_t(Ctx* c) {
   MsmWork* w = get_work(c);
   int rc = msm_queue_deferred<C>(c, w);
-  for (int k = 0; k < NSLOT; ++k) {
-    MsmSlot& sl = w->slot[(w->next + k) % NSLOT];
+  for (int k = 0; k < NSLOT_ALL; ++k) {
+    MsmSlot& sl = w->slot[k < NSLOT ? (w->next + k) % NSLOT : NSLOT + (w->jnext + k - NSLOT) % NSLOT_JOINT];
     int r2 = msm_retire<C>(c, sl);
     if (rc == KZG_OK) rc = r2;
   }
@@ -876,17 +1011,50 @@
     if (lens[p] > stride) return set_err(c, KZG_ERR_ARG, "kzg_commit: lens[p] > stride");
   }
   int rc = KZG_OK;
-  for (size_t p = 0; p < n_polys && rc == KZG_OK; ++p) {
-    uint64_t* o = out_xy + p * 2 * (F::NW / 2);
-    if (lens[p] == 0) {
-      memset(o, 0, 2 * F::NW * 4);
+  auto out_of = [&](size_t p) { return out_xy + p * 2 * (F::NW / 2); };
+  size_t p = 0;
+  while (p < n_polys && rc == KZG_OK) {
+    bool in_flight = false;
+    for (const MsmSlot& sl : w->slot) in_flight |= sl.pending;
+    const int cap = in_flight ? MSM_JOINT_MAX : 1;
+    size_t grp[MSM_JOINT_MAX];
+    int b = 0;
+    for (; p < n_polys && b < cap && rc == KZG_OK; ++p) {
+      if (lens[p] != 0) { grp[b++] = p; continue; }
+      memset(out_of(p), 0, 2 * F::NW * 4);
       out_inf[p] = 1;
       if (d_eval && out_eval) {
         if ((rc = KZG_HIP_RC(c, hipMemcpyAsync(out_eval, d_eval, 32, hipMemcpyDeviceToHost, c->stream)))) break;
         rc = KZG_HIP_RC(c, hipStreamSynchronize(c->stream));
       }
+    }
+    if (rc != KZG_OK || b == 0) break;
+    if (b >= 2) {
+      int slots[MSM_JOINT_MAX];
+      uint32_t ns[MSM_JOINT_MAX];
+      for (int j = 0; j < b && rc == KZG_OK; ++j) {
+        const int si = slots[j] = NSLOT + w->jnext;
+        w->jnext = (w->jnext + 1) % NSLOT_JOINT;
+        if ((rc = msm_retire<C>(c, w->slot[si]))) break;
+        const uint32_t* sc = d_scalars + grp[j] * stride * 8;
+        ns[j] = (uint32_t)lens[grp[j]];
+        rc = s->win_bits == 20 ? msm_enqueue_prep<C, 20>(c, s, sc, ns[j], w, si)
+                               : msm_enqueue_prep<C, 16>(c, s, sc, ns[j], w, si);
+      }
+      if (rc) break;
+      rc = s->win_bits == 20 ? msm_enqueue_joint<C, 20>(c, s, w, slots, ns, b)
+                             : msm_enqueue_joint<C, 16>(c, s, w, slots, ns, b);
+      if (rc) break;
+      for (int j = 0; j < b; ++j) {
+        MsmSlot& sl = w->slot[slots[j]];
+        sl.pending = true;
+        sl.out_eval = nullptr;
+        sl.out_xy = out_of(grp[j]);
+        sl.out_inf = out_inf + grp[j];
+      }
       continue;
     }
+    const size_t q = grp[0];
     const int si = w->next;
     MsmSlot& sl = w->slot[si];
     w->next = (w->next + 1) % NSLOT;
@@ -899,14 +1067,14 @@
         break;
       slot_eval = out_eval;
     }
-    const uint32_t* sc = d_scalars + p * stride * 8;
-    rc = s->win_bits == 20 ? msm_enqueue<C, 20>(c, s, sc, (uint32_t)lens[p], w, si)
-                           : msm_enqueue<C, 16>(c, s, sc, (uint32_t)lens[p], w, si);
+    const uint32_t* sc = d_scalars + q * stride * 8;
+    rc = s->win_bits == 20 ? msm_enqueue<C, 20>(c, s, sc, (uint32_t)lens[q], w, si)
+                           : msm_enqueue<C, 16>(c, s, sc, (uint32_t)lens[q], w, si);
     if (rc) break;
     sl.pending = true;
     sl.out_eval = slot_eval;
-    sl.out_xy = o;
-    sl.out_inf = out_inf + p;
+    sl.out_xy = out_of(q);
+    sl.out_inf = out_inf + q;
   }
   if (drain || rc != KZG_OK) {
     int r2 = commit_flush_t<C>(c);
diff --git a/kzg_snark_amd/csrc/msm_prep.h b/kzg_snark_amd/csrc/msm_prep.h
--- a/kzg_snark_amd/csrc/msm_prep.h
+++ b/kzg_snark_amd/csrc/msm_prep.h
@@ -9,4 +9,20 @@
                      uint32_t seg, void* ws, uint32_t* vals, uint32_t* bstart, uint32_t* order, uint32_t* slice_off,
                      uint32_t* chunk_counter, uint32_t* chunk_rank, uint32_t nchunk_max);
 
+struct MsmPolyDesc {
+  const uint32_t *vals, *bstart, *order, *slice_off, *chunk_rank;
+  uint32_t *partials, *buckets;
+  uint32_t total, pad;
+};
+constexpr int MSM_JOINT_MAX = 4;
+constexpr int MSM_JOINT_POLY_SHIFT = 28;
+struct MsmJointArgs {
+  MsmPolyDesc d[MSM_JOINT_MAX];
+};
+constexpr size_t MSM_JOINT_DESC_OFF = 64;
+constexpr size_t MSM_JOINT_LIST_OFF = MSM_JOINT_DESC_OFF + MSM_JOINT_MAX * sizeof(MsmPolyDesc);
+size_t msm_joint_bytes(uint32_t nchunk_max, uint32_t b);
+int msm_joint_enqueue(Ctx* c, hipStream_t sp, int win_bits, const MsmJointArgs& a, uint32_t b, uint32_t nchunk_max,
+                      void* joint);
+
 }
diff --git a/kzg_snark_amd/csrc/msm_prep.hip b/kzg_snark_amd/csrc/msm_prep.hip
--- a/kzg_snark_amd/csrc/msm_prep.hip
+++ b/kzg_snark_amd/csrc/msm_prep.hip
@@ -432,6 +432,60 @@
   chunk_rank[c] = lo;
 }
 
+
+__global__ __launch_bounds__(TPB) void prep_jdesc_kernel(MsmJointArgs a, uint32_t b, uint32_t nb, MsmPolyDesc* desc) {
+  side_priority();
+#pragma unroll
+  for (uint32_t p = 0; p < (uint32_t)MSM_JOINT_MAX; ++p)
+    if (threadIdx.x == p && p < b) {
+      MsmPolyDesc d = a.d[p];
+      d.total = d.slice_off[nb];
+      d.pad = 0;
+      desc[p] = d;
+    }
+}
+
+__device__ __forceinline__ uint32_t joint_class(const MsmPolyDesc& d, uint32_t c) {
+  const uint32_t r = d.chunk_rank[c], k = d.order[r];
+  const uint32_t len = d.bstart[k + 1] - d.bstart[k], ns = d.slice_off[r + 1] - d.slice_off[r];
+  return length_class((len + ns - 1) / ns);
+}
+
+__global__ __launch_bounds__(TPB) void prep_jcount_kernel(const MsmPolyDesc* desc, uint32_t* histj) {
+  side_priority();
+  __shared__ uint32_t hist[NCLS];
+  hist[threadIdx.x] = 0;
+  __syncthreads();
+  const MsmPolyDesc d = desc[blockIdx.y];
+  const uint32_t c = blockIdx.x * TPB + threadIdx.x;
+  if ((uint64_t)c * 64 < d.total) atomicAdd(&hist[joint_class(d, c)], 1u);
+  __syncthreads();
+  histj[(size_t)threadIdx.x * (gridDim.x * gridDim.y) + blockIdx.y * gridDim.x + blockIdx.x] = hist[threadIdx.x];
+}
+
+__global__ __launch_bounds__(TPB) void prep_jclasses_kernel(const uint32_t* class_total, uint32_t* class_start,
+                                                            uint32_t* head) {
+  side_priority();
+  __shared__ uint32_t sh[TPB];
+  const uint32_t v = class_total[threadIdx.x];
+  const uint32_t incl = block_inclusive_scan(v, sh);
+  class_start[threadIdx.x] = incl - v;
+  if (threadIdx.x == TPB - 1) { head[0] = 0; head[1] = 0; head[2] = incl; }
+}
+
+__global__ __launch_bounds__(TPB) void prep_jscatter_kernel(const MsmPolyDesc* desc, const uint32_t* histj,
+                                                            const uint32_t* class_start, uint32_t* list) {
+  side_priority();
+  __shared__ uint32_t cur[NCLS];
+  cur[threadIdx.x] = class_start[threadIdx.x] +
+                     histj[(size_t)threadIdx.x * (gridDim.x * gridDim.y) + blockIdx.y * gridDim.x + blockIdx.x];
+  __syncthreads();
+  const MsmPolyDesc d = desc[blockIdx.y];
+  const uint32_t c = blockIdx.x * TPB + threadIdx.x;
+  if ((uint64_t)c * 64 < d.total)
+    list[atomicAdd(&cur[joint_class(d, c)], 1u)] = (blockIdx.y << MSM_JOINT_POLY_SHIFT) | c;
+}
+
 size_t align256(size_t x) { return (x + 255) & ~(size_t)255; }
 
 template <int WB, int LOBV>
@@ -554,4 +608,44 @@
 #undef KZG_PREP_GO
 }
 
-}
+struct JointLayout {
+  uint32_t blocks;
+  size_t off_hist, off_class_total, off_class_start, total;
+  JointLayout(uint32_t nchunk_max, uint32_t b) {
+    blocks = (nchunk_max + TPB - 1) / TPB;
+    size_t t = align256(MSM_JOINT_LIST_OFF + (size_t)b * nchunk_max * 4);
+    auto take = [&](size_t bytes) { const size_t o = t; t += align256(bytes); return o; };
+    off_hist = take((size_t)NCLS * b * blocks * 4);
+    off_class_total = take(NCLS * 4);
+    off_class_start = take(NCLS * 4);
+    total = t;
+  }
+};
+
+size_t msm_joint_bytes(uint32_t nchunk_max, uint32_t b) { return JointLayout(nchunk_max, b).total; }
+
+int msm_joint_enqueue(Ctx* c, hipStream_t sp, int win_bits, const MsmJointArgs& a, uint32_t b, uint32_t nchunk_max,
+                      void* joint) {
+  if (b < 2 || b > (uint32_t)MSM_JOINT_MAX || nchunk_max >= (1u << MSM_JOINT_POLY_SHIFT))
+    return set_err(c, KZG_ERR_ARG, "msm_joint_enqueue: bad batch");
+  const JointLayout L(nchunk_max, b);
+  char* w = static_cast<char*>(joint);
+  auto* head = reinterpret_cast<uint32_t*>(w);
+  auto* desc = reinterpret_cast<MsmPolyDesc*>(w + MSM_JOINT_DESC_OFF);
+  auto* list = reinterpret_cast<uint32_t*>(w + MSM_JOINT_LIST_OFF);
+  auto* histj = reinterpret_cast<uint32_t*>(w + L.off_hist);
+  auto* class_total = reinterpret_cast<uint32_t*>(w + L.off_class_total);
+  auto* class_start = reinterpret_cast<uint32_t*>(w + L.off_class_start);
+  {
+    ProfScope ps(c, "msm_joint", sp);
+    hipLaunchKernelGGL(prep_jdesc_kernel, dim3(1), dim3(TPB), 0, sp, a, b, 1u << (win_bits - 1), desc);
+    hipLaunchKernelGGL(prep_jcount_kernel, dim3(L.blocks, b), dim3(TPB), 0, sp, desc, histj);
+    hipLaunchKernelGGL(prep_row_scan_kernel, dim3(NCLS), dim3(TPB), 0, sp, histj, L.blocks * b, class_total);
+    hipLaunchKernelGGL(prep_jclasses_kernel, dim3(1), dim3(TPB), 0, sp, class_total, class_start, head);
+    hipLaunchKernelGGL(prep_jscatter_kernel, dim3(L.blocks, b), dim3(TPB), 0, sp, desc, histj, class_start, list);
+  }
+  KZG_HIP(c, hipGetLastError());
+  return KZG_OK;
+}
+
+}
```

Measured after the change: 486.7 commits/s, median of 2. Within noise of the previous version (+1.1%).
